# ReubenBond/DistributedRateLimiting.Redis

Measured on AMD Instinct MI355X. Metric: acquire decisions/sec (node) at 100M keys, 1/2/4/8 GPU; % HBM roofline, higher is better.
Workload: dtype f64; 1 GPU; TokenBucket uniform keys, 2^26-request batches (config B); keys_total=100000000, keys_per_gpu=100000000, batch_per_gpu=67108864, period_ticks=10000000, partitioning=one GPU owns every key

## Files before the change

__graft_entry__.py:

```python
from __future__ import annotations

import os
import sys

ROOT = os.path.dirname(os.path.abspath(__file__))
if ROOT not in sys.path:
    sys.path.insert(0, ROOT)


def build() -> None:
    import importlib.util

    spec = importlib.util.spec_from_file_location(
        "_tbe_build", os.path.join(ROOT, "distributedratelimiting.redis_amd", "build.py"))
    mod = importlib.util.module_from_spec(spec)
    spec.loader.exec_module(mod)
    mod.build_engine(verbose=True)
    mod.build_host(verbose=True)
    from oracle.build import build_oracle

    build_oracle()
    spec = importlib.util.spec_from_file_location(
        "_host_test", os.path.join(ROOT, "tests", "test_host_cpp.py"))
    tmod = importlib.util.module_from_spec(spec)
    spec.loader.exec_module(tmod)
    tmod.build_host_test()
    import distributedratelimiting.redis_amd


def smoke() -> None:
    import numpy as np
    import torch

    from distributedratelimiting.redis_amd import TokenBucketEngine
    from oracle import cref, trace

    assert torch.cuda.is_available(), "smoke() needs a GPU"
    torch.cuda.set_device(0)
    n_keys, n = 10_000, 50_000
    token_limit, tokens_per_period, period_ticks = 20, 10, 10_000_000
    eng = TokenBucketEngine(n_keys, token_limit, tokens_per_period, period_ticks, device=0)
    ref = cref.CTokenBucket(n_keys, token_limit, eng_rate(tokens_per_period, period_ticks))
    for b in range(3):
        keys, permits, ts = trace.make_batch(0x5EED0001, n_keys, b, n, 200_000, 1, 3)
        g, r = eng.acquire_batch(keys, permits, ts)
        g_ref, r_ref = ref.acquire_batch(keys, permits, ts)
        assert np.array_equal(g, g_ref), f"granted mismatch in batch {b}"
        assert np.array_equal(r, r_ref), f"remaining mismatch in batch {b}"
    v, t = eng.export_state()
    v_ref, t_ref = ref.export_state()
    touched = t_ref != np.iinfo(np.int64).min
    assert np.array_equal(t, t_ref)
    assert np.array_equal(v[touched].view(np.uint64), v_ref[touched].view(np.uint64))
    eng.close()
    print(f"smoke ok: {3 * n} decisions bit-exact vs oracle, grant rate {g.mean():.3f}")


def eng_rate(tokens_per_period: int, period_ticks: int) -> float:
    from distributedratelimiting.redis_amd import fill_rate

    return fill_rate(tokens_per_period, period_ticks)


if __name__ == "__main__":
    build()
    if len(sys.argv) > 1 and sys.argv[1] == "smoke":
        smoke()
```

distributedratelimiting.redis_amd/build.py:

```python
from __future__ import annotations

import os
import shutil
import subprocess
import sys

HERE = os.path.dirname(os.path.realpath(__file__))
ROOT = os.path.dirname(HERE)
SOURCES = [os.path.join(HERE, "csrc", n) for n in ("tbe_engine.hip", "tbe_tools.hip", "tbe_cluster.hip", "tbe_strdir.hip")]
DEPS = SOURCES + [os.path.join(HERE, "csrc", n) for n in ("tbe_device.hpp", "tbe_codec.hpp", "tbe_numfmt.hpp", "tbe_hash.hpp")] + \
    [os.path.join(ROOT, "include", n) for n in ("tbe.h", "tbe_tools.h", "tbe_cluster.h", "tbe_strdir.h")]
LIB = os.path.join(HERE, "libtbe.so")
ARCH = "gfx950"
HIPCC_FLAGS = ["-O3", "-std=c++17", "-ffp-contract=off", "-fno-fast-math", "-fPIC", "-shared",
               "-Wall", "-Wno-unused-result", f"--offload-arch={ARCH}"]


def hipcc() -> str:
    for cand in (os.environ.get("HIPCC"), shutil.which("hipcc"), "/opt/rocm/bin/hipcc"):
        if cand and os.path.exists(cand):
            return cand
    raise FileNotFoundError("hipcc not found")


def _digest(deps, flags) -> str:
    import hashlib
    h = hashlib.sha256(" ".join(flags).encode())
    for d in deps:
        with open(d, "rb") as f:
            h.update(os.path.basename(d).encode() + b"\0" + f.read())
    return h.hexdigest()


def up_to_date(target: str, deps, flags=()) -> bool:
    stamp = target + ".sha256"
    if not (os.path.exists(target) and os.path.exists(stamp)):
        return False
    with open(stamp) as f:
        return f.read().strip() == _digest(deps, flags)


def _stamp(target: str, deps, flags=()) -> None:
    with open(target + ".sha256", "w") as f:
        f.write(_digest(deps, flags) + "\n")


def build_engine(force: bool = False, verbose: bool = False, defines=(), out: str = LIB) -> str:
    flags = HIPCC_FLAGS + [f"-D{d}" for d in defines]
    if not force and up_to_date(out, DEPS, flags):
        if verbose:
            print(f"build: {os.path.basename(out)} up to date (sources sha256 {_digest(DEPS, flags)[:12]})",
                  file=sys.stderr)
        return out
    cmd = [hipcc()] + flags + ["-I", os.path.join(ROOT, "include"), "-o", out + ".tmp"] + SOURCES
    if verbose:
        print(" ".join(cmd), file=sys.stderr)
    subprocess.run(cmd, check=True)
    os.replace(out + ".tmp", out)
    _stamp(out, DEPS, flags)
    return out


HOST_SRC = os.path.join(HERE, "host", "rate_limiting.cpp")
HOST_DEPS = [HOST_SRC, os.path.join(HERE, "host", "rate_limiting.hpp"), os.path.join(ROOT, "include", "tbe.h")]
HOST_LIB = os.path.join(HERE, "libtbe_host.so")
CXX_FLAGS = ["-O2", "-std=c++17", "-Wall", "-Wextra", "-Wno-unused-parameter", "-pthread"]


def build_host(force: bool = False, verbose: bool = False) -> str:
    build_engine(verbose=verbose)
    if not force and up_to_date(HOST_LIB, HOST_DEPS + [LIB], CXX_FLAGS):
        return HOST_LIB
    cmd = ["g++"] + CXX_FLAGS + ["-fPIC", "-shared", "-I", os.path.join(ROOT, "include"),
                                 "-o", HOST_LIB + ".tmp", HOST_SRC, "-L", HERE, "-ltbe",
                                 "-Wl,-rpath,$ORIGIN"]
    if verbose:
        print(" ".join(cmd), file=sys.stderr)
    subprocess.run(cmd, check=True)
    os.replace(HOST_LIB + ".tmp", HOST_LIB)
    _stamp(HOST_LIB, HOST_DEPS + [LIB], CXX_FLAGS)
    return HOST_LIB


if __name__ == "__main__":
    print(build_engine(force="--force" in sys.argv, verbose=True))
    print(build_host(force="--force" in sys.argv, verbose=True))
```

distributedratelimiting.redis_amd/csrc/tbe_codec.hpp:

```cpp
#pragma once
#include <cstdint>

#if defined(__HIPCC__)
#define TBE_CODEC_FN __host__ __device__ __forceinline__
#else
#define TBE_CODEC_FN inline
#endif

struct PackFmt {
    uint64_t kmask;
    int32_t kb;
    int32_t pb;
    int32_t pc_max;
    int32_t wb;
    int32_t n0;
    int32_t rb;
    int32_t w0;
};
TBE_CODEC_FN uint32_t pack_rec32(uint32_t pkey, int32_t p, int64_t ts, int64_t tbase, const PackFmt &F, bool &esc) {
    const uint32_t pc = (uint32_t)(p < 0 ? 0 : (p > F.pc_max ? F.pc_max : p));
    const uint64_t d = (uint64_t)ts - (uint64_t)tbase;
    const bool fits = ts >= tbase && (d >> F.w0) == 0;
    esc = !fits;
    return (pkey & ((1u << F.rb) - 1u)) | (pc << F.rb) | ((uint32_t)!fits << (F.rb + F.pb)) |
           (fits ? (uint32_t)d << (F.rb + F.pb + 1) : 0u);
}

struct FoldFmt {
    int32_t on;
    int32_t n0;
    int32_t rb, pb, pw, tw;
    uint32_t nb;
    uint32_t region_bits;
    uint32_t n_hi;
};
TBE_CODEC_FN uint64_t fold_rec32(uint32_t r32, uint32_t pos, int64_t tbase0, int64_t tbase1, const PackFmt &F,
                           const FoldFmt &G) {
    const uint64_t row = r32 & ((1u << F.rb) - 1u);
    const uint64_t pc = (r32 >> F.rb) & ((1u << F.pb) - 1u);
    const bool esc0 = (r32 >> (F.rb + F.pb)) & 1u;
    const int64_t ts = (int64_t)((uint64_t)tbase0 + (uint64_t)(r32 >> (F.rb + F.pb + 1)));
    const uint64_t d = (uint64_t)ts - (uint64_t)tbase1;
    const bool fits = !esc0 && ts >= tbase1 && (d >> G.tw) == 0;
    return row | (pc << G.rb) | ((uint64_t)!fits << (G.rb + G.pb)) | ((uint64_t)pos << (G.rb + G.pb + 1)) |
           ((fits ? d : 0ull) << (G.rb + G.pb + 1 + G.pw));
}

struct Pass1Codec {
    uint32_t low_mask;
    uint32_t s_esc;
    uint32_t s_pos;
    uint32_t s_time;
    uint64_t dconst;
};
TBE_CODEC_FN bool pass1_codec_ok(const PackFmt &F, const FoldFmt &G) {
    return F.n0 && G.pw >= 1 && G.pw <= 32 && F.rb == G.rb && F.pb == G.pb && F.w0 == 32 - F.rb - F.pb - 1 &&
           F.w0 >= 1 && G.tw == 64 - G.rb - G.pb - 1 - G.pw && G.tw >= F.w0;
}
TBE_CODEC_FN Pass1Codec pass1_codec(const PackFmt &F, const FoldFmt &G, bool have_ts) {
    Pass1Codec C;
    C.s_esc = (uint32_t)(F.rb + F.pb);
    C.s_pos = C.s_esc + 1u;
    C.s_time = C.s_pos + (uint32_t)G.pw;
    C.low_mask = (1u << C.s_pos) - 1u;
    C.dconst = have_ts ? (1ull << (G.tw - 1)) - (1ull << (F.w0 - 1)) : 0ull;
    return C;
}
TBE_CODEC_FN uint64_t fold_rec32_codec(uint32_t r32, uint32_t pos, const Pass1Codec &C) {
    const bool esc0 = (r32 >> C.s_esc) & 1u;
    const uint64_t d = (uint64_t)(r32 >> C.s_pos) + C.dconst;
    const uint32_t plo = pos << C.s_pos, phi = pos >> (32u - C.s_pos);
    return ((uint64_t)phi << 32 | ((r32 & C.low_mask) | plo)) | ((esc0 ? 0ull : d) << C.s_time);
}
```

distributedratelimiting.redis_amd/csrc/tbe_device.hpp:

```cpp
#pragma once

#include <hip/hip_runtime.h>
#include <stdint.h>

#pragma clang fp contract(off)

namespace tbe {

constexpr int kBlock = 256;
constexpr int kWaves = kBlock / 64;
constexpr int kDigitBits = 8;
constexpr int kDigits = 1 << kDigitBits;
constexpr int64_t kAbsent = INT64_MIN;

struct __attribute__((aligned(16))) Slot {
    double v;
    int64_t t_us;
};

__device__ __forceinline__ double lua_max(double a, double b) { return (b > a) ? b : a; }
__device__ __forceinline__ double lua_min(double a, double b) { return (b < a) ? b : a; }

__device__ __forceinline__ void split_ts(int64_t ts_us, int64_t &sec, int64_t &usec) {
    int64_t s = (int64_t)((double)ts_us * 1e-6);
    int64_t r = ts_us - s * 1000000;
    if (r < 0) {
        s -= 1;
        r += 1000000;
    } else if (r >= 1000000) {
        s += 1;
        r -= 1000000;
    }
    sec = s;
    usec = r;
}

__device__ __forceinline__ double new_t_of(int64_t ts_us) {
    int64_t sec, usec;
    split_ts(ts_us, sec, usec);
    const double x = (double)usec;
    const double rcp = 1.0 / 1000000.0;
    const double q0 = x * rcp;
    const double r = __builtin_fma(-q0, 1000000.0, x);
    const double q = __builtin_fma(r, rcp, q0);
    return (double)sec + q;
}

struct TbParams {
    double cap;
    double rate;
    int64_t ttl_ms;
};

struct ReqTime {
    double new_t;
    int64_t exp_lt;
    int64_t ts;
};
__device__ __forceinline__ ReqTime req_time(int64_t ts_us, int64_t ttl_ms) {
    ReqTime r;
    r.new_t = new_t_of(ts_us);
    r.exp_lt = (ts_us / 1000 - ttl_ms) * 1000;
    r.ts = ts_us;
    return r;
}

struct TimeBase {
    int64_t tbase;
    int64_t e0;
    uint32_t sec0;
    uint32_t usec0;
    uint32_t r0;
    uint32_t ok;
};
constexpr uint64_t kRelMax = 0xFFFFFFFFull - 1000000ull;
__host__ __device__ inline TimeBase time_base(int64_t tbase, int64_t ttl_ms) {
    TimeBase b{tbase, 0, 0, 0, 0, 0};
    if (tbase < 0) return b;
    const int64_t sec0 = tbase / 1000000;
    if (sec0 > (int64_t)0xFFFFFFFFll - 10000) return b;
    b.sec0 = (uint32_t)sec0;
    b.usec0 = (uint32_t)(tbase - sec0 * 1000000);
    b.r0 = (uint32_t)(tbase % 1000);
    b.e0 = (tbase / 1000 - ttl_ms) * 1000;
    b.ok = 1;
    return b;
}
__device__ __forceinline__ ReqTime req_time_rel(int64_t ts_us, const TimeBase &B, int64_t ttl_ms) {
    const uint64_t d = (uint64_t)ts_us - (uint64_t)B.tbase;
    if (!B.ok || ts_us < B.tbase || d > kRelMax) return req_time(ts_us, ttl_ms);
    const uint32_t u = B.usec0 + (uint32_t)d;
    const uint32_t s1 = u / 1000000u;
    const uint32_t usec = u - s1 * 1000000u;
    const uint32_t sec = B.sec0 + s1;
    const double x = (double)usec;
    const double rcp = 1.0 / 1000000.0;
    const double q0 = x * rcp;
    const double r = __builtin_fma(-q0, 1000000.0, x);
    const double q = __builtin_fma(r, rcp, q0);
    ReqTime rt;
    rt.new_t = (double)sec + q;
    rt.exp_lt = B.e0 + (int64_t)((B.r0 + (uint32_t)d) / 1000u) * 1000;
    rt.ts = ts_us;
    return rt;
}
#ifndef TBE_ABSENT_BASE
#define TBE_ABSENT_BASE 1
#endif
__device__ __forceinline__ int64_t absent_t(const TimeBase &B) { return TBE_ABSENT_BASE ? B.tbase : 0; }

__device__ __forceinline__ uint32_t tb_step_ft(Slot &row, double ft, int32_t permits,
                                               const ReqTime &rq, const TbParams &P, bool &modified) {
    const bool had = row.t_us != kAbsent;
    const bool expired = had && row.t_us < rq.exp_lt;
    const bool present = had && !expired;
    const double pv = present ? row.v : P.cap;
    const double pt = present ? ft : rq.new_t;
    const double delta_t = lua_max(0.0, rq.new_t - pt);
    const double fill = delta_t * P.rate;
    double x = lua_max(0.0, lua_min(P.cap, pv + fill));
    const double p = (double)permits;
    const bool granted = x >= p;
    if (granted) {
        x = x - p;
        row.v = x;
        row.t_us = rq.ts;
    } else if (expired) {
        row.v = P.cap;
        row.t_us = kAbsent;
    }
    modified = granted || expired;
    return (granted ? 0x80000000u : 0u) | (uint32_t)(int32_t)x;
}

__device__ __forceinline__ uint32_t tb_step(Slot &row, int32_t permits, const ReqTime &rq,
                                            const TbParams &P, bool &modified) {
    const double ft = new_t_of(row.t_us == kAbsent ? 0 : row.t_us);
    return tb_step_ft(row, ft, permits, rq, P, modified);
}

__device__ __forceinline__ uint32_t tb_acquire(Slot &s, int32_t permits, int64_t ts_us,
                                               const TbParams &P, bool &modified) {
    return tb_step(s, permits, req_time(ts_us, P.ttl_ms), P, modified);
}

template <typename T>
__device__ __forceinline__ T ld_nt(const T *p) { return __builtin_nontemporal_load(p); }
template <typename T>
__device__ __forceinline__ void st_nt(T *p, T v) { __builtin_nontemporal_store(v, p); }

__device__ __forceinline__ uint32_t xcd_swizzle(uint32_t b, uint32_t nblk) {
    const uint32_t xcd = b & 7u, q = nblk >> 3, r = nblk & 7u;
    return (xcd < r ? xcd * (q + 1) : r * (q + 1) + (xcd - r) * q) + (b >> 3);
}

__device__ __forceinline__ uint64_t lanemask_lt() {
    const int lane = threadIdx.x & 63;
    return (lane == 0) ? 0ull : ((~0ull) >> (64 - lane));
}

template <int BLOCK>
__device__ __forceinline__ uint32_t block_excl_scan(uint32_t x, uint32_t *wsum, uint32_t *total) {
    constexpr int W = BLOCK / 64;
    const int lane = threadIdx.x & 63, w = threadIdx.x >> 6;
    uint32_t v = x;
#pragma unroll
    for (int o = 1; o < 64; o <<= 1) {
        const uint32_t y = __shfl_up(v, o, 64);
        if (lane >= o) v += y;
    }
    if (lane == 63) wsum[w] = v;
    __syncthreads();
    uint32_t pre = 0, tot = 0;
#pragma unroll
    for (int j = 0; j < W; ++j) {
        const uint32_t s = wsum[j];
        pre += (j < w) ? s : 0u;
        tot += s;
    }
    *total = tot;
    __syncthreads();
    return pre + v - x;
}

#ifndef TBE_WAVE_MATCH
#define TBE_WAVE_MATCH 1
#endif
__device__ __forceinline__ uint64_t digit_peers(uint32_t key, int shift, uint64_t vmask) {
#if TBE_WAVE_MATCH
    const uint32_t dg = (key >> shift) & (kDigits - 1);
    uint32_t dlo = 0, dhi = 0;
#pragma unroll
    for (int b = 0; b < kDigitBits; ++b) {
        const uint32_t sb = (uint32_t)__builtin_amdgcn_sbfe((int)dg, (uint32_t)b, 1u);
        const uint64_t m = __builtin_amdgcn_uicmp(sb, 0u, 33);
        dlo |= (uint32_t)m ^ sb;
        dhi |= (uint32_t)(m >> 32) ^ sb;
    }
    return vmask & ~(((uint64_t)dhi << 32) | dlo);
#else
    const uint32_t dg = (key >> shift) & (kDigits - 1);
    uint64_t peers = vmask;
#pragma unroll
    for (int b = 0; b < kDigitBits; ++b) {
        const bool bit = (dg >> b) & 1u;
        const uint64_t m = __ballot(bit);
        peers &= bit ? m : ~m;
    }
    return peers;
#endif
}

template <int BLOCK>
struct RankLds {
    static constexpr int W = BLOCK / 64;
    static constexpr int PARTS = BLOCK / kDigits;
    uint32_t lstart[kDigits];
    uint32_t part[PARTS][kDigits];
    uint32_t wsum[W];
};

template <int BLOCK, int ITEMS>
__device__ __forceinline__ void rank_tile(const uint32_t (&key)[ITEMS], int shift, int nvalid,
                                          RankLds<BLOCK> &L, uint16_t *cnt,
                                          uint32_t (&lpos)[ITEMS]) {
#define TBE_DIG(it) ((key[it] >> shift) & (kDigits - 1))
    constexpr int W = BLOCK / 64;
    constexpr int COL = ITEMS * W;
    static_assert(BLOCK % kDigits == 0, "whole digit columns per thread group");
    const int tid = threadIdx.x, w = tid >> 6;
    {
        uint4 *z = reinterpret_cast<uint4 *>(cnt);
        const uint4 zero = {0u, 0u, 0u, 0u};
        for (int i = tid; i < COL * kDigits * 2 / 16; i += BLOCK) z[i] = zero;
    }
    __syncthreads();
    const uint64_t lt = lanemask_lt();
#pragma unroll
    for (int it = 0; it < ITEMS; ++it) {
        const int e = it * BLOCK + tid;
        const bool valid = e < nvalid;
        const uint32_t dg = TBE_DIG(it);
        const uint64_t peers = digit_peers(key[it], shift, __ballot(valid));
        lpos[it] = (uint32_t)__popcll(peers & lt);
        if (valid && lpos[it] == 0) cnt[(it * W + w) * kDigits + dg] = (uint16_t)__popcll(peers);
    }
    __syncthreads();
    constexpr int PARTS = BLOCK / kDigits;
    static_assert(COL % PARTS == 0, "column splits evenly");
    constexpr int SEG = COL / PARTS;
    const int d = tid & (kDigits - 1);
    const int part = tid / kDigits;
    uint32_t s = 0;
#pragma unroll 8
    for (int j = part * SEG; j < (part + 1) * SEG; ++j) {
        const uint32_t c = cnt[j * kDigits + d];
        cnt[j * kDigits + d] = (uint16_t)s;
        s += c;
    }
    L.part[part][d] = s;
    __syncthreads();
    uint32_t off = 0, total = 0;
#pragma unroll
    for (int q = 0; q < PARTS; ++q) {
        const uint32_t v = L.part[q][d];
        off += (q < part) ? v : 0u;
        total += v;
    }
    if (part > 0) {
#pragma unroll 8
        for (int j = part * SEG; j < (part + 1) * SEG; ++j)
            cnt[j * kDigits + d] = (uint16_t)(cnt[j * kDigits + d] + off);
    }
    {
        uint32_t all;
        const uint32_t ex = block_excl_scan<BLOCK>(part == 0 ? total : 0u, L.wsum, &all);
        if (part == 0) L.lstart[d] = ex;
    }
    __syncthreads();
#pragma unroll
    for (int it = 0; it < ITEMS; ++it)
        lpos[it] += L.lstart[TBE_DIG(it)] + cnt[(it * W + w) * kDigits + TBE_DIG(it)];
#undef TBE_DIG
}

template <int BLOCK, int ITEMS>
__device__ __forceinline__ int wb_elem(int it) {
    return (int)((threadIdx.x >> 6) * (64 * ITEMS) + it * 64 + (threadIdx.x & 63));
}

template <int BLOCK, int ITEMS, bool FULL = false>
__device__ __forceinline__ void rank_tile_wb(const uint32_t (&key)[ITEMS], int shift, int nvalid,
                                             RankLds<BLOCK> &L, uint32_t *wcnt, uint32_t (&lpos)[ITEMS]) {
    constexpr int W = BLOCK / 64;
    const int tid = threadIdx.x, w = tid >> 6, lane = tid & 63;
    uint32_t *mine = wcnt + w * kDigits;
#pragma unroll
    for (int i = lane; i < kDigits; i += 64) mine[i] = 0;
    __builtin_amdgcn_fence(__ATOMIC_RELEASE, "wavefront");
    const uint64_t lt = lanemask_lt();
#pragma unroll
    for (int it = 0; it < ITEMS; ++it) {
        const int e = wb_elem<BLOCK, ITEMS>(it);
        const bool valid = FULL || e < nvalid;
        const uint32_t dg = (key[it] >> shift) & (kDigits - 1);
        const uint64_t peers = digit_peers(key[it], shift, FULL ? ~0ull : __ballot(valid));
        const int leader = (FULL || peers) ? __ffsll((long long)peers) - 1 : lane;
        uint32_t old = 0;
        if (valid && leader == lane) old = atomicAdd(&mine[dg], (uint32_t)__popcll(peers));
        old = __shfl(old, leader, 64);
        lpos[it] = old + (uint32_t)__popcll(peers & lt);
    }
    __syncthreads();
    uint32_t tot = 0;
    if (tid < kDigits) {
#pragma unroll
        for (int v = 0; v < W; ++v) {
            const uint32_t c = wcnt[v * kDigits + tid];
            wcnt[v * kDigits + tid] = tot;
            tot += c;
        }
    }
    {
        uint32_t all;
        const uint32_t ex = block_excl_scan<BLOCK>(tid < kDigits ? tot : 0u, L.wsum, &all);
        if (tid < kDigits) L.lstart[tid] = ex;
    }
    __syncthreads();
#pragma unroll
    for (int it = 0; it < ITEMS; ++it) {
        const uint32_t dg = (key[it] >> shift) & (kDigits - 1);
        lpos[it] += L.lstart[dg] + mine[dg];
    }
}

}
```

distributedratelimiting.redis_amd/csrc/tbe_engine.hip:

```cpp
#include <hip/hip_runtime.h>

#include <algorithm>
#include <cmath>
#include <cstdarg>
#include <cstdio>
#include <cstdlib>
#include <cstring>
#include <new>
#include <string>
#include <thread>
#include <tuple>
#include <type_traits>
#include <vector>

#include "../../include/tbe.h"
#include "tbe_device.hpp"
#include "tbe_codec.hpp"
#include "tbe_numfmt.hpp"

#pragma clang fp contract(off)

using namespace tbe;

namespace {

#ifndef TBE_NO_NT
#define LD_P(p) ld_nt(p)
#define ST_PERM(p, v) st_nt((p), (v))
#define LD_U(p) ld_nt(p)
#define ST_U(p, v) st_nt((p), (v))
#define ST_S(p, v) slot_store_nt((p), (v))
#else
#define LD_P(p) (*(p))
#define ST_PERM(p, v) (*(p) = (v))
#define LD_U(p) (*(p))
#define ST_U(p, v) (*(p) = (v))
#define ST_S(p, v) (*(p) = (v))
#endif
#define LD_F(p) (*(p))
#define ST_F(p, v) (*(p) = (v))

#ifndef TBE_PART_BLOCK
#define TBE_PART_BLOCK 512
#endif
#ifndef TBE_PART_ITEMS
#define TBE_PART_ITEMS 8
#endif
constexpr int kPartBlock = TBE_PART_BLOCK;
constexpr int kPartItems = TBE_PART_ITEMS;
constexpr int kTile = kPartBlock * kPartItems;
#ifndef TBE_UN_BLOCK
#define TBE_UN_BLOCK 1024
#endif
#ifndef TBE_UN_ITEMS
#define TBE_UN_ITEMS 8
#endif
constexpr int kUnBlock = TBE_UN_BLOCK;
constexpr int kUnItems = TBE_UN_ITEMS;
constexpr int kUnTile = kUnBlock * kUnItems;
#ifndef TBE_FULL_TILE
#define TBE_FULL_TILE 1
#endif
#ifndef TBE_HIST_BLOCKS
#define TBE_HIST_BLOCKS 1024
#endif
constexpr int kMaxHistBlocks = TBE_HIST_BLOCKS;
static_assert(kMaxHistBlocks % 256 == 0, "k_colscan reads kMaxHistBlocks / 256 blocks per thread");
constexpr int kMaxRBits = 11;

constexpr uint32_t kHotKeysMax = 1024;
#ifndef TBE_HOT_SLOT_BITS
#define TBE_HOT_SLOT_BITS 12
#endif
constexpr uint32_t kHotSlots = 1u << TBE_HOT_SLOT_BITS;
static_assert(kHotSlots >= 2 * kHotKeysMax, "hot table load factor <= 1/2");
constexpr uint32_t kHotEmpty = 0xFFFFFFFFu;
constexpr uint32_t kHotMin = 2048;
constexpr uint32_t kHotCandMax = 4096;

struct HotSet {
    uint32_t count;
    uint32_t n_cand;
    uint32_t key[kHotKeysMax];
    uint64_t cand[kHotCandMax];
    uint64_t slot[kHotSlots];
};

__device__ __forceinline__ uint32_t hot_hash(uint32_t key) { return (key * 0x9E3779B1u) >> (32 - TBE_HOT_SLOT_BITS); }
constexpr uint64_t kHotSlotEmpty = 0xFFFFFFFFFFFFFFFFull;
constexpr uint32_t kHotHalf = kHotSlots / 2;
__device__ __forceinline__ uint32_t hot_h1(uint32_t key) { return (key * 0x9E3779B1u) >> (33 - TBE_HOT_SLOT_BITS); }
__device__ __forceinline__ uint32_t hot_h2(uint32_t key) {
    uint32_t x = (key ^ (key >> 16)) * 0x85EBCA6Bu;
    x ^= x >> 13;
    return kHotHalf + ((x * 0xC2B2AE35u) >> (33 - TBE_HOT_SLOT_BITS));
}

constexpr uint32_t kHotLds = kHotSlots;
template <int BLOCK>
__device__ __forceinline__ bool hot_load(const HotSet *__restrict__ hot, uint64_t *slots) {
    const bool any = hot != nullptr && hot->count != 0;
    if (any)
        for (int j = threadIdx.x; j < (int)kHotSlots; j += BLOCK) slots[j] = hot->slot[j];
    __syncthreads();
    return any;
}
__device__ __forceinline__ const uint64_t *hot_table(const HotSet *__restrict__, const uint64_t *lds) {
    return lds;
}

__device__ __forceinline__ uint32_t hot_sortkey(uint32_t key, const uint64_t *slots, uint32_t nb,
                                                int r_bits) {
    const uint64_t v1 = slots[hot_h1(key)], v2 = slots[hot_h2(key)];
    if ((uint32_t)v1 == key) return (nb + (uint32_t)(v1 >> 32)) << r_bits;
    if ((uint32_t)v2 == key) return (nb + (uint32_t)(v2 >> 32)) << r_bits;
    return key;
    uint32_t h = hot_hash(key);
    for (;;) {
        const uint64_t v = slots[h];
        const uint32_t k = (uint32_t)v;
        if (k == key) return (nb + (uint32_t)(v >> 32)) << r_bits;
        if (k == kHotEmpty) return key;
        h = (h + 1) & (kHotSlots - 1);
    }
}

template <int N, typename KeyT>
__device__ __forceinline__ void hot_sortkeys(const KeyT (&kv)[N], const uint64_t *slots, uint32_t nb,
                                             int r_bits, uint32_t (&sk)[N]) {
    constexpr int G = N < 4 ? N : 4;
    static_assert(N % G == 0, "groups of G requests");
#pragma unroll
    for (int g = 0; g < N; g += G) {
        uint64_t v1[G], v2[G];
#pragma unroll
        for (int u = 0; u < G; ++u) {
            v1[u] = slots[hot_h1((uint32_t)kv[g + u])];
            v2[u] = slots[hot_h2((uint32_t)kv[g + u])];
        }
#pragma unroll
        for (int u = 0; u < G; ++u) {
            const uint32_t key = (uint32_t)kv[g + u];
            const bool in1 = (uint32_t)v1[u] == key;
            const uint64_t v = in1 ? v1[u] : v2[u];
            sk[g + u] = (in1 || (uint32_t)v2[u] == key) ? (nb + (uint32_t)(v >> 32)) << r_bits : key;
        }
    }
    return;
    uint64_t v[N];
#pragma unroll
    for (int it = 0; it < N; ++it) v[it] = slots[hot_hash((uint32_t)kv[it])];
#pragma unroll
    for (int it = 0; it < N; ++it) {
        const uint32_t key = (uint32_t)kv[it];
        const uint32_t k = (uint32_t)v[it];
        if (k == key) sk[it] = (nb + (uint32_t)(v[it] >> 32)) << r_bits;
        else if (k == kHotEmpty) sk[it] = key;
        else sk[it] = hot_sortkey(key, slots, nb, r_bits);
    }
}

constexpr int kHBlock = 512;
constexpr int kHItems = kTile / kHBlock;
#ifndef TBE_HIST_AHEAD
#define TBE_HIST_AHEAD 1
#endif
#ifndef TBE_HIST_WAVES
#define TBE_HIST_WAVES 8
#endif
#ifndef TBE_HIST_HOT_WAVES
#define TBE_HIST_HOT_WAVES 6
#endif
template <typename KeyT, bool HOT = false>
__global__ __launch_bounds__(kHBlock, HOT ? TBE_HIST_HOT_WAVES : TBE_HIST_WAVES) void k_hist(const KeyT *__restrict__ keys, uint64_t n,
                                                  int shift, uint32_t tiles_per_blk,
                                                  uint32_t ntiles, uint32_t *__restrict__ tileprefix,
                                                  uint32_t *__restrict__ blocksum, uint64_t n_keys,
                                                  uint32_t *__restrict__ err, int validate,
                                                  uint64_t kmask, const HotSet *__restrict__ hot = nullptr,
                                                  uint32_t nb = 0, int r_bits = 0,
                                                  uint32_t *__restrict__ bcount = nullptr,
                                                  int lowbits = 0, uint32_t nbt = 0,
                                                  uint8_t *__restrict__ dig_out = nullptr) {
    __shared__ uint32_t h8[kDigits * 8];
    __shared__ uint32_t tile_lo[2];
    static_assert(kHBlock == 2 * kDigits && kDigits * 8 == 4 * kHBlock, "two threads per digit; 4 counters each");
    __shared__ uint64_t hs[HOT ? kHotLds : 1];
    const int tid = threadIdx.x;
    const bool dig = tid < kDigits;
    const bool any_hot = HOT && hot_load<kHBlock>(hot, hs);
    const uint32_t t0 = blockIdx.x * tiles_per_blk;
    const uint32_t t1 = min(t0 + tiles_per_blk, ntiles);
    uint32_t run = 0;
    uint32_t acc = 0, acc_lo = 0;
    bool bad = false;
    KeyT kn[kHItems];
#if TBE_HIST_AHEAD >= 2
    KeyT kn2[kHItems];
#endif
    auto load_into = [&](KeyT (&dst)[kHItems], uint32_t t) {
#pragma unroll
        for (int it = 0; it < kHItems; ++it) {
            const uint64_t i = (uint64_t)t * kTile + it * kHBlock + tid;
            dst[it] = (t < t1 && i < n) ? LD_P(keys + i) : (KeyT)0;
        }
    };
    load_into(kn, t0);
#if TBE_HIST_AHEAD >= 2
    load_into(kn2, t0 + 1);
#endif
    for (uint32_t t = t0; t < t1; ++t) {
        KeyT kv[kHItems];
#pragma unroll
        for (int it = 0; it < kHItems; ++it) kv[it] = kn[it];
#if TBE_HIST_AHEAD >= 2
#pragma unroll
        for (int it = 0; it < kHItems; ++it) kn[it] = kn2[it];
        load_into(kn2, t + 2);
#else
        load_into(kn, t + 1);
#endif
#pragma unroll
        for (int u = 0; u < 4; ++u) h8[u * kHBlock + tid] = 0;
        __syncthreads();
        const uint64_t base = (uint64_t)t * kTile;
        const uint64_t last = min<uint64_t>(base + kTile, n) - 1;
        uint32_t skv[kHItems];
        if (HOT && any_hot) {
            hot_sortkeys<kHItems>(kv, hot_table(hot, hs), nb, r_bits, skv);
        } else {
#pragma unroll
            for (int it = 0; it < kHItems; ++it) skv[it] = (uint32_t)((uint64_t)kv[it] & kmask);
        }
#pragma unroll
        for (int it = 0; it < kHItems; ++it) {
            const uint64_t i = base + it * kHBlock + tid;
            const bool valid = i < n;
            const uint32_t sk = skv[it];
            const uint32_t d = (sk >> shift) & (kDigits - 1);
            const uint64_t vmask = __ballot(valid);
            const uint32_t d0 = __shfl(d, vmask ? __ffsll((long long)vmask) - 1 : 0, 64);
            if (__all(!valid || d == d0)) {
                if (vmask && (vmask & lanemask_lt()) == 0 && valid) atomicAdd(&h8[d0 * 8], (uint32_t)__popcll(vmask));
            } else {
                if (valid) atomicAdd(&h8[d * 8 + (tid & 7)], 1u);
            }
            if (dig_out && valid) dig_out[i] = (uint8_t)d;
            if (valid) {
                bad |= validate && ((uint64_t)kv[it] >= n_keys);
                if (bcount && (i == base || i == last)) {
                    tile_lo[i == last] = lowbits ? (sk >> r_bits) & ((1u << lowbits) - 1u) : 0u;
                    if (i == base && i == last) tile_lo[0] = tile_lo[1];
                }
            }
        }
        __syncthreads();
        uint32_t c = 0;
        if (dig) {
#pragma unroll
            for (int u = 0; u < 8; ++u) c += h8[tid * 8 + ((u + tid) & 7)];
            tileprefix[(uint64_t)t * kDigits + tid] = run;
            run += c;
        }
        if (bcount) {
            const uint32_t lo0 = tile_lo[0], lo1 = tile_lo[1];
            if (lo0 == lo1) {
                if (dig) {
                    if (lo0 != acc_lo) {
                        const uint32_t bk = ((uint32_t)tid << lowbits) | acc_lo;
                        if (acc && bk < nbt) atomicAdd(&bcount[bk], acc);
                        acc = 0;
                        acc_lo = lo0;
                    }
                    acc += c;
                }
            } else if (lo1 - lo0 < 8) {
                __syncthreads();
#pragma unroll
                for (int u = 0; u < 4; ++u) h8[u * kHBlock + tid] = 0;
                __syncthreads();
#pragma unroll
                for (int it = 0; it < kHItems; ++it) {
                    const uint64_t i = base + it * kHBlock + tid;
                    const uint32_t bk = skv[it] >> r_bits;
                    if (i < n) atomicAdd(&h8[((bk & ((1u << lowbits) - 1u)) - lo0) * kDigits + ((bk >> lowbits) & (kDigits - 1))], 1u);
                }
                __syncthreads();
                if (dig) {
                    for (uint32_t u = 0; u <= lo1 - lo0; ++u) {
                        const uint32_t cnt = h8[u * kDigits + tid];
                        const uint32_t bk = ((uint32_t)tid << lowbits) | (lo0 + u);
                        if (cnt && bk < nbt) atomicAdd(&bcount[bk], cnt);
                    }
                }
            } else {
#pragma unroll
                for (int it = 0; it < kHItems; ++it) {
                    const uint64_t i = base + it * kHBlock + tid;
                    const uint32_t bk = skv[it] >> r_bits;
                    if (i < n && bk < nbt) atomicAdd(&bcount[bk], 1u);
                }
            }
        }
        __syncthreads();
    }
    if (bcount && dig) {
        const uint32_t bk = ((uint32_t)tid << lowbits) | acc_lo;
        if (acc && bk < nbt) atomicAdd(&bcount[bk], acc);
    }
    if (dig) blocksum[(uint64_t)blockIdx.x * kDigits + tid] = run;
    if (__any(bad) && (tid & 63) == 0) atomicOr(err, 1u);
}

__global__ __launch_bounds__(kHBlock, TBE_HIST_WAVES) void k_hist_dig(
    const uint8_t *__restrict__ dig, uint64_t n, uint32_t tiles_per_blk, uint32_t ntiles,
    uint32_t *__restrict__ tileprefix, uint32_t *__restrict__ blocksum,
    const uint32_t *__restrict__ dtot0, uint32_t *__restrict__ bcount, uint32_t nbt) {
    __shared__ uint32_t h8[kDigits * 8];
    __shared__ uint32_t dstart[kDigits + 1];
    __shared__ uint32_t wsum[kHBlock / 64];
    __shared__ uint32_t tlo[kHBlock];
    static_assert(kHBlock == 2 * kDigits && kDigits * 8 == 4 * kHBlock, "two threads per digit; 4 counters each");
    static_assert(kHItems % 8 == 0, "8-byte loads");
    constexpr int kW = kHItems / 8;
    const int tid = threadIdx.x;
    const bool own = tid < kDigits;
    {
        uint32_t all;
        const uint32_t pre = block_excl_scan<kHBlock>(own ? dtot0[tid] : 0u, wsum, &all);
        if (own) dstart[tid] = pre;
        if (tid == 0) dstart[kDigits] = 0xFFFFFFFFu;
    }
    auto d0_of = [&](uint32_t i) {
        uint32_t lo = 0, hi = kDigits;
        while (hi - lo > 1) {
            const uint32_t mid = (lo + hi) >> 1;
            if (dstart[mid] <= i) lo = mid;
            else hi = mid;
        }
        return lo;
    };
    const uint32_t t0 = blockIdx.x * tiles_per_blk;
    const uint32_t t1 = min(t0 + tiles_per_blk, ntiles);
    uint32_t run = 0, acc = 0, acc_lo = 0;
    auto load = [&](uint32_t t, uint64_t (&dst)[kW]) {
#pragma unroll
        for (int q = 0; q < kW; ++q) {
            const uint64_t i = (uint64_t)t * kTile + (uint64_t)tid * kHItems + 8 * q;
            uint64_t v = 0;
            if (t < t1 && i + 8 <= n) {
                v = LD_P(reinterpret_cast<const uint64_t *>(dig + i));
            } else if (t < t1) {
                for (int u = 0; i + u < n; ++u) v |= (uint64_t)dig[i + u] << (8 * u);
            }
            dst[q] = v;
        }
    };
    uint64_t vn[kW];
    load(t0, vn);
    __syncthreads();
    for (uint32_t t = t0; t < t1; ++t) {
        uint64_t vw[kW];
#pragma unroll
        for (int q = 0; q < kW; ++q) vw[q] = vn[q];
        load(t + 1, vn);
#pragma unroll
        for (int u = 0; u < 4; ++u) h8[u * kHBlock + tid] = 0;
        const uint64_t base = (uint64_t)t * kTile;
        const uint32_t tk = (t - t0) % (kHBlock / 2);
        if (tk == 0) {
            const uint32_t tt = t + (uint32_t)(tid >> 1);
            if (tt < t1) {
                const uint64_t b = (uint64_t)tt * kTile;
                tlo[tid] = d0_of((uint32_t)((tid & 1) ? min<uint64_t>(b + kTile, n) - 1 : b));
            }
        }
        __syncthreads();
        if (TBE_FULL_TILE && base + kTile <= n) {
#pragma unroll
            for (int u = 0; u < kHItems; ++u) {
                const uint32_t d = (uint32_t)(vw[u >> 3] >> (8 * (u & 7))) & (kDigits - 1);
                const uint32_t dw = (uint32_t)__builtin_amdgcn_readfirstlane((int)d);
                if (__all(d == dw)) {
                    if ((tid & 63) == 0) atomicAdd(&h8[dw * 8], 64u);
                } else {
                    atomicAdd(&h8[d * 8 + (tid & 7)], 1u);
                }
            }
        } else {
            const uint32_t nv = (uint32_t)(n - base);
#pragma unroll
            for (int u = 0; u < kHItems; ++u) {
                const bool valid = (uint32_t)(tid * kHItems + u) < nv;
                const uint32_t d = (uint32_t)(vw[u >> 3] >> (8 * (u & 7))) & (kDigits - 1);
                const uint64_t vmask = __ballot(valid);
                const uint32_t dw = __shfl(d, vmask ? __ffsll((long long)vmask) - 1 : 0, 64);
                if (__all(!valid || d == dw)) {
                    if (vmask && (vmask & lanemask_lt()) == 0 && valid) atomicAdd(&h8[dw * 8], (uint32_t)__popcll(vmask));
                } else if (valid) {
                    atomicAdd(&h8[d * 8 + (tid & 7)], 1u);
                }
            }
        }
        __syncthreads();
        uint32_t c = 0;
        if (own) {
#pragma unroll
            for (int u = 0; u < 8; ++u) c += h8[tid * 8 + ((u + tid) & 7)];
            tileprefix[(uint64_t)t * kDigits + tid] = run;
            run += c;
        }
        const uint32_t lo0 = tlo[2 * tk], lo1 = tlo[2 * tk + 1];
        if (lo0 == lo1) {
            if (own) {
                if (lo0 != acc_lo) {
                    const uint32_t bk = ((uint32_t)tid << kDigitBits) | acc_lo;
                    if (acc && bk < nbt) atomicAdd(&bcount[bk], acc);
                    acc = 0;
                    acc_lo = lo0;
                }
                acc += c;
            }
        } else if (lo1 - lo0 < 8) {
            __syncthreads();
#pragma unroll
            for (int u = 0; u < 4; ++u) h8[u * kHBlock + tid] = 0;
            __syncthreads();
#pragma unroll
            for (int u = 0; u < kHItems; ++u) {
                const uint64_t i = base + (uint64_t)tid * kHItems + u;
                if (i >= n) continue;
                uint32_t lo = 0;
                for (uint32_t x = 1; x <= lo1 - lo0; ++x) lo += dstart[lo0 + x] <= (uint32_t)i;
                const uint32_t d = (uint32_t)(vw[u >> 3] >> (8 * (u & 7))) & (kDigits - 1);
                atomicAdd(&h8[lo * kDigits + d], 1u);
            }
            __syncthreads();
            if (own) {
                for (uint32_t u = 0; u <= lo1 - lo0; ++u) {
                    const uint32_t cnt = h8[u * kDigits + tid];
                    const uint32_t bk = ((uint32_t)tid << kDigitBits) | (lo0 + u);
                    if (cnt && bk < nbt) atomicAdd(&bcount[bk], cnt);
                }
            }
        } else {
#pragma unroll
            for (int u = 0; u < kHItems; ++u) {
                const uint64_t i = base + (uint64_t)tid * kHItems + u;
                if (i >= n) continue;
                const uint32_t bk = (((uint32_t)(vw[u >> 3] >> (8 * (u & 7))) & (kDigits - 1)) << kDigitBits) | d0_of((uint32_t)i);
                if (bk < nbt) atomicAdd(&bcount[bk], 1u);
            }
        }
        __syncthreads();
    }
    if (own) {
        const uint32_t bk = ((uint32_t)tid << kDigitBits) | acc_lo;
        if (acc && bk < nbt) atomicAdd(&bcount[bk], acc);
        blocksum[(uint64_t)blockIdx.x * kDigits + tid] = run;
    }
}

__global__ __launch_bounds__(kBlock) void k_colscan(const uint32_t *__restrict__ blocksum,
                                                    uint32_t nblk,
                                                    uint32_t *__restrict__ blockprefix,
                                                    uint32_t *__restrict__ digit_total) {
    __shared__ uint32_t wsum[kWaves];
    const int d = blockIdx.x, tid = threadIdx.x;
    constexpr int PER = kMaxHistBlocks / kBlock;
    uint32_t c[PER], s = 0;
#pragma unroll
    for (int u = 0; u < PER; ++u) {
        const uint32_t j = tid * PER + u;
        c[u] = (j < nblk) ? blocksum[(uint64_t)j * kDigits + d] : 0u;
        s += c[u];
    }
    uint32_t total;
    uint32_t pre = block_excl_scan<kBlock>(s, wsum, &total);
#pragma unroll
    for (int u = 0; u < PER; ++u) {
        const uint32_t j = tid * PER + u;
        if (j < nblk) blockprefix[(uint64_t)j * kDigits + d] = pre;
        pre += c[u];
    }
    if (tid == 0) digit_total[d] = total;
}

template <int BLOCK>
__device__ __forceinline__ void tile_offsets(uint32_t tile, uint32_t tiles_per_blk,
                                             const uint32_t *__restrict__ tileprefix,
                                             const uint32_t *__restrict__ blockprefix,
                                             const uint32_t *__restrict__ digit_total,
                                             uint32_t *goff, uint32_t *wsum) {
    const int tid = threadIdx.x;
    uint32_t tot = (tid < kDigits) ? digit_total[tid] : 0u;
    uint32_t all;
    const uint32_t base = block_excl_scan<BLOCK>(tot, wsum, &all);
    if (tid < kDigits)
        goff[tid] = base + blockprefix[(uint64_t)(tile / tiles_per_blk) * kDigits + tid] +
                    tileprefix[(uint64_t)tile * kDigits + tid];
}

template <typename KeyIn, bool IDX, bool TS = true>
__global__ __launch_bounds__(kPartBlock) void k_scatter(
    const KeyIn *__restrict__ kin, const int32_t *__restrict__ pin, const int64_t *__restrict__ tin,
    const uint32_t *__restrict__ iin, uint64_t n, int shift, const uint32_t *__restrict__ tileprefix,
    const uint32_t *__restrict__ blockprefix, const uint32_t *__restrict__ digit_total,
    uint32_t tiles_per_blk, uint32_t *__restrict__ kout, int32_t *__restrict__ pout,
    int64_t *__restrict__ tout, uint32_t *__restrict__ iout, uint32_t *__restrict__ perm,
    uint32_t *__restrict__ err, int validate) {
    __shared__ RankLds<kPartBlock> L;
    __shared__ uint32_t goff[kDigits];
    __shared__ uint64_t stage[kTile];
    static_assert(kPartItems * (kPartBlock / 64) * kDigits * 2 <= kTile * 8, "cnt fits in stage");

    const int tid = threadIdx.x;
    const uint32_t tile = xcd_swizzle(blockIdx.x, gridDim.x);
    const uint64_t base = (uint64_t)tile * kTile;
    const int nvalid = (int)min<uint64_t>(kTile, n - base);

    uint32_t key[kPartItems], lpos[kPartItems];
    int32_t pm[kPartItems];
    int64_t tv[kPartItems];
#pragma unroll
    for (int it = 0; it < kPartItems; ++it) {
        const int e = it * kPartBlock + tid;
        const bool v = e < nvalid;
        key[it] = v ? (uint32_t)kin[base + e] : 0u;
        pm[it] = v ? pin[base + e] : 0;
        tv[it] = (v && TS) ? tin[base + e] : 0;
    }
    tile_offsets<kPartBlock>(tile, tiles_per_blk, tileprefix, blockprefix, digit_total, goff, L.wsum);
    rank_tile<kPartBlock, kPartItems>(key, shift, nvalid, L, reinterpret_cast<uint16_t *>(stage), lpos);
    __syncthreads();

    bool bad = false;
#pragma unroll
    for (int it = 0; it < kPartItems; ++it) {
        const int e = it * kPartBlock + tid;
        if (e < nvalid) {
            const uint32_t d = (key[it] >> shift) & (kDigits - 1);
            bad |= validate && (pm[it] < 0 || tv[it] < 0);
            stage[lpos[it]] = ((uint64_t)key[it] << 32) | (uint32_t)pm[it];
            perm[base + e] = goff[d] + lpos[it] - L.lstart[d];
        }
    }
    __syncthreads();
    uint32_t gpos[kPartItems];
#pragma unroll
    for (int it = 0; it < kPartItems; ++it) {
        const int j = it * kPartBlock + tid;
        if (j < nvalid) {
            const uint64_t s = stage[j];
            const uint32_t k = (uint32_t)(s >> 32);
            const uint32_t d = (k >> shift) & (kDigits - 1);
            gpos[it] = goff[d] + (uint32_t)j - L.lstart[d];
            kout[gpos[it]] = k;
            pout[gpos[it]] = (int32_t)(uint32_t)s;
        }
    }
    if (TS) {
        __syncthreads();
#pragma unroll
        for (int it = 0; it < kPartItems; ++it) {
            const int e = it * kPartBlock + tid;
            if (e < nvalid) stage[lpos[it]] = (uint64_t)tv[it];
        }
        __syncthreads();
#pragma unroll
        for (int it = 0; it < kPartItems; ++it) {
            const int j = it * kPartBlock + tid;
            if (j < nvalid) tout[gpos[it]] = (int64_t)stage[j];
        }
    }
    if (IDX) {
        uint32_t *stage32 = reinterpret_cast<uint32_t *>(stage);
        uint32_t iv[kPartItems];
#pragma unroll
        for (int it = 0; it < kPartItems; ++it) {
            const int e = it * kPartBlock + tid;
            iv[it] = (e < nvalid) ? (iin ? iin[base + e] : (uint32_t)(base + e)) : 0u;
        }
        __syncthreads();
#pragma unroll
        for (int it = 0; it < kPartItems; ++it) {
            const int e = it * kPartBlock + tid;
            if (e < nvalid) stage32[lpos[it]] = iv[it];
        }
        __syncthreads();
#pragma unroll
        for (int it = 0; it < kPartItems; ++it) {
            const int j = it * kPartBlock + tid;
            if (j < nvalid) iout[gpos[it]] = stage32[j];
        }
    }
    if (validate && __any(bad) && (tid & 63) == 0) atomicOr(err, 1u);
}

constexpr int kScanPer = 16;
__global__ __launch_bounds__(1024) void k_bscan(const uint32_t *__restrict__ bcount, uint32_t nbt,
                                                uint32_t *__restrict__ bstart, uint32_t nb = 0,
                                                uint32_t wide_min = 0, uint32_t *__restrict__ dlist = nullptr) {
    __shared__ uint32_t tile[1024 * (kScanPer + 1)];
    auto pad = [](uint32_t j) { return (j / kScanPer) * (kScanPer + 1) + (j % kScanPer); };
    __shared__ uint32_t wsum[16];
    __shared__ uint32_t n_dense;
    if (threadIdx.x == 0) n_dense = 0;
    const uint32_t t = threadIdx.x;
    constexpr uint32_t kRow = 1024 * kScanPer;
    constexpr int kGroup = 4;
    uint32_t carry = 0;
    for (uint32_t g0 = 0; g0 < nbt; g0 += kGroup * kRow) {
        uint32_t ld[kGroup][kScanPer];
#pragma unroll
        for (int r = 0; r < kGroup; ++r)
#pragma unroll
            for (int k = 0; k < kScanPer; ++k) {
                const uint32_t j = g0 + r * kRow + k * 1024 + t;
                ld[r][k] = j < nbt ? bcount[j] : 0u;
            }
#pragma unroll
        for (int r = 0; r < kGroup; ++r) {
            const uint32_t r0 = g0 + r * kRow;
            if (r0 >= nbt) break;
#pragma unroll
            for (int k = 0; k < kScanPer; ++k) tile[pad(k * 1024 + t)] = ld[r][k];
            __syncthreads();
            uint32_t v[kScanPer], sum = 0;
#pragma unroll
            for (int k = 0; k < kScanPer; ++k) {
                v[k] = tile[t * (kScanPer + 1) + k];
                sum += v[k];
            }
            if (dlist) {
#pragma unroll
                for (int k = 0; k < kScanPer; ++k) {
                    const uint32_t bk = r0 + t * kScanPer + k;
                    if (bk < nb && v[k] >= wide_min) dlist[1 + atomicAdd(&n_dense, 1u)] = bk;
                }
            }
            uint32_t total;
            uint32_t pre = carry + block_excl_scan<1024>(sum, wsum, &total);
#pragma unroll
            for (int k = 0; k < kScanPer; ++k) {
                tile[t * (kScanPer + 1) + k] = pre;
                pre += v[k];
            }
            __syncthreads();
#pragma unroll
            for (int k = 0; k < kScanPer; ++k) {
                const uint32_t j = r0 + k * 1024 + t;
                if (j < nbt) bstart[j] = tile[pad(k * 1024 + t)];
            }
            carry += total;
            __syncthreads();
        }
    }
    if (t == 0) bstart[nbt] = carry;
    if (dlist) {
        __syncthreads();
        if (t == 0) dlist[0] = n_dense;
    }
}

constexpr int kBsPer = 4;
constexpr uint32_t kBsTile = 1024u * kBsPer;
constexpr uint32_t kBsMaxBlocks = 64;
__global__ __launch_bounds__(1024) void k_bscan_lb(const uint32_t *__restrict__ bcount, uint32_t nbt,
                                                   uint32_t *__restrict__ bstart,
                                                   unsigned long long *__restrict__ flags, uint32_t tag,
                                                   uint32_t nb = 0, uint32_t wide_min = 0,
                                                   uint32_t *__restrict__ dlist = nullptr) {
    __shared__ uint32_t wsum[16];
    __shared__ uint32_t excl;
    const uint32_t t = threadIdx.x, blk = blockIdx.x;
    const uint32_t b0 = blk * kBsTile + t * kBsPer;
    uint32_t v[kBsPer];
#pragma unroll
    for (int k = 0; k < kBsPer; ++k) v[k] = (b0 + k < nbt) ? bcount[b0 + k] : 0u;
    if (dlist) {
#pragma unroll
        for (int k = 0; k < kBsPer; ++k)
            if (b0 + k < nb && v[k] >= wide_min) dlist[1 + atomicAdd(dlist, 1u)] = b0 + k;
    }
    uint32_t sum = 0;
#pragma unroll
    for (int k = 0; k < kBsPer; ++k) sum += v[k];
    uint32_t total;
    const uint32_t pre = block_excl_scan<1024>(sum, wsum, &total);
    if (t == 0)
        __hip_atomic_store(&flags[blk], ((unsigned long long)tag << 32) | total, __ATOMIC_RELEASE,
                           __HIP_MEMORY_SCOPE_AGENT);
    if (t < 64) {
        uint32_t acc = 0;
        for (uint32_t j0 = 0; j0 < blk; j0 += 64) {
            const uint32_t j = j0 + t;
            uint32_t val = 0;
            if (j < blk) {
                unsigned long long f;
                do {
                    f = __hip_atomic_load(&flags[j], __ATOMIC_ACQUIRE, __HIP_MEMORY_SCOPE_AGENT);
                } while ((uint32_t)(f >> 32) != tag);
                val = (uint32_t)f;
            }
#pragma unroll
            for (int o = 32; o > 0; o >>= 1) val += __shfl_xor(val, o, 64);
            acc += val;
        }
        if (t == 0) excl = acc;
    }
    __syncthreads();
    uint32_t run = excl + pre;
#pragma unroll
    for (int k = 0; k < kBsPer; ++k) {
        if (b0 + k < nbt) bstart[b0 + k] = run;
        run += v[k];
    }
    if (blk == gridDim.x - 1 && t == 0) bstart[nbt] = excl + total;
}

__device__ __forceinline__ int64_t pack_base32(const int64_t *__restrict__ ts, const PackFmt &F) {
    return ts[0] - ((int64_t)1 << (F.w0 - 1));
}
__device__ __forceinline__ int64_t pack_base(const int64_t *__restrict__ ts, const PackFmt &F) {
    return ts[0] - ((int64_t)1 << (F.wb - 1));
}
#ifndef TBE_REL_BASE
#define TBE_REL_BASE 1
#endif
__device__ __forceinline__ int64_t rel_base(const int64_t *__restrict__ ts, const PackFmt &F) {
#if TBE_REL_BASE
    (void)F;
    const int64_t b = ts[0] - ((int64_t)1 << 31);
    return b > 0 ? b : 0;
#else
    return pack_base(ts, F);
#endif
}
__device__ __forceinline__ uint64_t pack_rec(uint64_t key, int32_t p, int64_t ts, uint64_t idx,
                                             int64_t tbase, const PackFmt &F) {
    const uint64_t pc = (uint64_t)(p < 0 ? 0 : (p > F.pc_max ? F.pc_max : p));
    const uint64_t d = (uint64_t)ts - (uint64_t)tbase;
    const bool fits = ts >= tbase && (d >> F.wb) == 0;
    const uint64_t pay = fits ? d : idx;
    return (key & F.kmask) | (pc << F.kb) | ((uint64_t)!fits << (F.kb + F.pb)) |
           (pay << (F.kb + F.pb + 1));
}
__device__ __forceinline__ void unpack_rec(uint64_t rec, const int64_t *__restrict__ ts_orig,
                                           int64_t tbase, const PackFmt &F, uint32_t &key,
                                           int32_t &p, int64_t &ts) {
    key = (uint32_t)(rec & F.kmask);
    p = (int32_t)((rec >> F.kb) & ((1ull << F.pb) - 1));
    const uint64_t pay = rec >> (F.kb + F.pb + 1);
    ts = ((rec >> (F.kb + F.pb)) & 1) ? ts_orig[pay] : (int64_t)((uint64_t)tbase + pay);
}

__device__ __forceinline__ int64_t fold_base(const int64_t *__restrict__ ts, const FoldFmt &G) {
    return ts[0] - ((int64_t)1 << (G.tw - 1));
}
__device__ __forceinline__ uint64_t fold_rec(uint64_t rec0, uint32_t pos, int64_t tbase0, int64_t tbase1,
                                             const PackFmt &F, const FoldFmt &G) {
    const uint64_t row = rec0 & ((1ull << G.rb) - 1);
    const uint64_t pc = (rec0 >> F.kb) & ((1ull << F.pb) - 1);
    const bool esc0 = (rec0 >> (F.kb + F.pb)) & 1;
    const int64_t ts = (int64_t)((uint64_t)tbase0 + (rec0 >> (F.kb + F.pb + 1)));
    const uint64_t d = (uint64_t)ts - (uint64_t)tbase1;
    const bool fits = !esc0 && ts >= tbase1 && (d >> G.tw) == 0;
    return row | (pc << G.rb) | ((uint64_t)!fits << (G.rb + G.pb)) | ((uint64_t)pos << (G.rb + G.pb + 1)) |
           ((fits ? d : 0ull) << (G.rb + G.pb + 1 + G.pw));
}
__device__ __forceinline__ void unfold_rec(uint64_t rec, const FoldFmt &G, int64_t tbase1,
                                           const uint64_t *__restrict__ rec0, const int64_t *__restrict__ ts_orig,
                                           int64_t tbase0, const PackFmt &F, uint32_t &row, int32_t &p,
                                           int64_t &ts, uint32_t &pos) {
    row = (uint32_t)(rec & ((1ull << G.rb) - 1));
    p = (int32_t)((rec >> G.rb) & ((1ull << G.pb) - 1));
    pos = (uint32_t)((rec >> (G.rb + G.pb + 1)) & ((1ull << G.pw) - 1));
    if ((rec >> (G.rb + G.pb)) & 1) {
        if (G.n0) {
            ts = (int64_t)rec0[pos];
        } else {
            uint32_t k;
            int32_t p0;
            unpack_rec(rec0[pos], ts_orig, tbase0, F, k, p0, ts);
        }
    } else {
        ts = (int64_t)((uint64_t)tbase1 + (rec >> (G.rb + G.pb + 1 + G.pw)));
    }
}
__device__ __forceinline__ uint32_t fold_bucket_at(const FoldFmt &G, uint32_t blk) {
    if (!G.on) return blk;
    const uint32_t x = blk & 7u, s = blk >> 3;
    const uint32_t j = s / G.n_hi, hi = s - j * G.n_hi;
    return (hi << G.region_bits) | (x + 8u * j);
}
__device__ __forceinline__ uint32_t fold_bucket(const FoldFmt &G) { return fold_bucket_at(G, blockIdx.x); }
__device__ __forceinline__ void fold_input(uint64_t rec, uint32_t q, const FoldFmt &G, int64_t tbase1,
                                           const uint64_t *__restrict__ rec0, const int64_t *__restrict__ ts_orig,
                                           int64_t tbase0, const PackFmt &F, uint32_t rmask, uint32_t &row,
                                           int32_t &p, int64_t &ts, uint32_t &pos) {
    if (G.on) {
        unfold_rec(rec, G, tbase1, rec0, ts_orig, tbase0, F, row, p, ts, pos);
    } else {
        uint32_t k;
        unpack_rec(rec, ts_orig, tbase0, F, k, p, ts);
        row = k & rmask;
        pos = q;
    }
}

#ifndef TBE_FOLD_FAM
#define TBE_FOLD_FAM 1
#endif
template <int FAM>
__device__ __forceinline__ void fold_input_fam(uint64_t rec, uint32_t q, const FoldFmt &G, int64_t tbase1,
                                               const uint64_t *__restrict__ rec0,
                                               const int64_t *__restrict__ ts_orig, int64_t tbase0,
                                               const PackFmt &F, uint32_t rmask, uint32_t &row, int32_t &p,
                                               int64_t &ts, uint32_t &pos) {
    if (FAM < 0) {
        fold_input(rec, q, G, tbase1, rec0, ts_orig, tbase0, F, rmask, row, p, ts, pos);
    } else if (FAM == 0) {
        uint32_t k;
        unpack_rec(rec, ts_orig, tbase0, F, k, p, ts);
        row = k & rmask;
        pos = q;
    } else {
        row = (uint32_t)(rec & ((1ull << G.rb) - 1));
        p = (int32_t)((rec >> G.rb) & ((1ull << G.pb) - 1));
        pos = (uint32_t)((rec >> (G.rb + G.pb + 1)) & ((1ull << G.pw) - 1));
        if ((rec >> (G.rb + G.pb)) & 1) {
            if (FAM == 1) {
                ts = (int64_t)rec0[pos];
            } else {
                uint32_t k;
                int32_t p0;
                unpack_rec(rec0[pos], ts_orig, tbase0, F, k, p0, ts);
            }
        } else {
            ts = (int64_t)((uint64_t)tbase1 + (rec >> (G.rb + G.pb + 1 + G.pw)));
        }
    }
}

#ifndef TBE_BSCAN_LB
#define TBE_BSCAN_LB 1
#endif
#ifndef TBE_NARROW0
#define TBE_NARROW0 1
#endif
#ifndef TBE_SCATTER0_WAVES
#define TBE_SCATTER0_WAVES 1
#endif
#ifndef TBE_PASS1_CODEC
#define TBE_PASS1_CODEC 1
#endif
constexpr int kLastWaves = 3 * (kPartBlock / 64) / 4;
template <bool FIRST, bool HOT = false, bool IDX = false, bool NOTS = false, bool LAST = false, int FAM = -1>
__global__ __launch_bounds__(kPartBlock, FIRST ? TBE_SCATTER0_WAVES : (FAM >= 0 ? kLastWaves : 1)) void k_scatter_rec(
    const uint64_t *__restrict__ kin, const int32_t *__restrict__ pin, const int64_t *__restrict__ tin,
    const uint64_t *__restrict__ rin, uint64_t n, int shift, PackFmt F,
    const uint32_t *__restrict__ tileprefix, const uint32_t *__restrict__ blockprefix,
    const uint32_t *__restrict__ digit_total, uint32_t tiles_per_blk, uint64_t *__restrict__ rout,
    uint32_t *__restrict__ perm, uint32_t *__restrict__ err, const HotSet *__restrict__ hot = nullptr,
    uint32_t nb = 0, int r_bits = 0, const uint32_t *__restrict__ iin = nullptr,
    uint32_t *__restrict__ iout = nullptr, FoldFmt G = FoldFmt{}, uint8_t *__restrict__ dig_next = nullptr,
    const uint8_t *__restrict__ din = nullptr, int64_t *__restrict__ ts0 = nullptr, Pass1Codec C = Pass1Codec{}) {
    static_assert(!(FIRST && LAST), "fold records come from a pass after the first");
    static_assert(FAM < 0 || LAST, "the record family is fixed only for the last pass");
    const bool n0 = FAM < 0 ? F.n0 != 0 : FAM == 1;
    __shared__ RankLds<kPartBlock> L;
    __shared__ uint32_t goff[kDigits];
    __shared__ uint64_t stage[kTile];
    __shared__ uint16_t stage_e[LAST ? kTile : 1];
    __shared__ uint64_t hs[HOT ? kHotLds : 1];
    static_assert(kPartItems * (kPartBlock / 64) * kDigits * 2 <= kTile * 8, "cnt fits in stage");

    const int tid = threadIdx.x;
    const uint32_t tile = xcd_swizzle(blockIdx.x, gridDim.x);
    const uint64_t base = (uint64_t)tile * kTile;
    const int nv = (int)min((uint32_t)kTile, (uint32_t)(n - base));

    auto body = [&](auto full) {
        constexpr bool FULL = decltype(full)::value;
        const int nvalid = nv;
        uint64_t rec[kPartItems];
        uint32_t key[kPartItems], lpos[kPartItems];
        bool bad = false;
        bool any_hot = false;
        int64_t tv_keep[FIRST ? kPartItems : 1];
        if (FIRST) {
            uint64_t kv[kPartItems];
            int32_t pv[kPartItems];
            int64_t tv[kPartItems];
#pragma unroll
            for (int it = 0; it < kPartItems; ++it) {
                const int e = wb_elem<kPartBlock, kPartItems>(it);
                const bool v = (FULL || e < nvalid);
                kv[it] = v ? LD_P(kin + base + e) : 0ull;
                pv[it] = v ? LD_P(pin + base + e) : 0;
                tv[it] = NOTS ? -1 : (v ? LD_P(tin + base + e) : 0);
            }
            any_hot = HOT && hot_load<kPartBlock>(hot, hs);
            const int64_t tbase = NOTS ? 0 : (n0 ? pack_base32(tin, F) : pack_base(tin, F));
            uint32_t skv[kPartItems];
            if (HOT && any_hot) {
                hot_sortkeys<kPartItems>(kv, hot_table(hot, hs), nb, r_bits, skv);
            } else {
#pragma unroll
                for (int it = 0; it < kPartItems; ++it) skv[it] = (uint32_t)(kv[it] & F.kmask);
            }
#pragma unroll
            for (int it = 0; it < kPartItems; ++it) {
                const int e = wb_elem<kPartBlock, kPartItems>(it);
                bad |= (FULL || e < nvalid) && (pv[it] < 0 || (!NOTS && tv[it] < 0));
                if (n0) {
                    bool esc = false;
                    const uint32_t r32 =
                        NOTS ? (skv[it] & ((1u << F.rb) - 1u)) |
                                   ((uint32_t)(pv[it] < 0 ? 0 : (pv[it] > F.pc_max ? F.pc_max : pv[it])) << F.rb)
                             : pack_rec32(skv[it], pv[it], tv[it], tbase, F, esc);
                    rec[it] = (uint64_t)r32 | ((uint64_t)((skv[it] >> shift) & (kDigits - 1)) << 32) |
                              ((uint64_t)((skv[it] >> (shift + kDigitBits)) & (kDigits - 1)) << 40) |
                              ((uint64_t)esc << 48);
                } else {
                    rec[it] = pack_rec(skv[it], pv[it], tv[it], base + e, tbase, F);
                }
                key[it] = skv[it];
                tv_keep[FIRST ? it : 0] = tv[it];
            }
        } else {
            if (n0) {
                const uint32_t *rin32 = reinterpret_cast<const uint32_t *>(rin);
                uint8_t dv[kPartItems];
#pragma unroll
                for (int it = 0; it < kPartItems; ++it) {
                    const int e = wb_elem<kPartBlock, kPartItems>(it);
                    rec[it] = (FULL || e < nvalid) ? (uint64_t)LD_P(rin32 + base + e) : 0ull;
                    dv[it] = (FULL || e < nvalid) ? din[base + e] : (uint8_t)0;
                }
#pragma unroll
                for (int it = 0; it < kPartItems; ++it) {
                    key[it] = (uint32_t)dv[it] << shift;
                    rec[it] |= (uint64_t)dv[it] << 32;
                }
            } else {
#pragma unroll
                for (int it = 0; it < kPartItems; ++it) {
                    const int e = wb_elem<kPartBlock, kPartItems>(it);
                    rec[it] = (FULL || e < nvalid) ? LD_P(rin + base + e) : 0ull;
                    key[it] = (uint32_t)(rec[it] & F.kmask);
                }
            }
        }
        tile_offsets<kPartBlock>(tile, tiles_per_blk, tileprefix, blockprefix, digit_total, goff, L.wsum);
        rank_tile_wb<kPartBlock, kPartItems, FULL>(key, shift, nvalid, L, reinterpret_cast<uint32_t *>(stage), lpos);
        int64_t tbase0 = 0, tbase1 = 0;
        if (LAST && FAM != 1 && tin) {
            tbase0 = n0 ? pack_base32(tin, F) : pack_base(tin, F);
            tbase1 = fold_base(tin, G);
        }
        __syncthreads();
#pragma unroll
        for (int it = 0; it < kPartItems; ++it) {
            const int e = wb_elem<kPartBlock, kPartItems>(it);
            if (FULL || e < nvalid) {
                const uint32_t d = (key[it] >> shift) & (kDigits - 1);
                stage[lpos[it]] = n0 ? (rec[it] & 0x0000FFFFFFFFFFFFull) : rec[it];
                if (LAST)
                    stage_e[lpos[it]] = (uint16_t)e;
                else if (perm)
                    ST_PERM(perm + base + e, goff[d] + lpos[it] - L.lstart[d]);
                if (FIRST && n0 && ((rec[it] >> 48) & 1u))
                    ts0[goff[d] + lpos[it] - L.lstart[d]] = tv_keep[FIRST ? it : 0];
            }
        }
        __syncthreads();
        uint32_t gpos[kPartItems];
#pragma unroll
        for (int it = 0; it < kPartItems; ++it) {
            const int j = it * kPartBlock + tid;
            if (FULL || j < nvalid) {
                const uint64_t s = stage[j];
                const uint32_t d = n0 ? (uint32_t)(s >> 32) & (kDigits - 1)
                                      : ((uint32_t)(s & F.kmask) >> shift) & (kDigits - 1);
                gpos[it] = goff[d] + (uint32_t)j - L.lstart[d];
                if (n0 && !LAST)
                    reinterpret_cast<uint32_t *>(rout)[gpos[it]] = (uint32_t)s;
                else if (n0)
                    rout[gpos[it]] = FAM == 1 ? fold_rec32_codec((uint32_t)s, (uint32_t)(base + stage_e[j]), C)
                                              : fold_rec32((uint32_t)s, (uint32_t)(base + stage_e[j]), tbase0, tbase1, F, G);
                else
                    rout[gpos[it]] = LAST ? fold_rec(s, (uint32_t)(base + stage_e[j]), tbase0, tbase1, F, G) : s;
                if (!LAST && dig_next)
                    dig_next[gpos[it]] = n0 ? (uint8_t)(s >> 40)
                                            : (uint8_t)(((uint32_t)(s & F.kmask) >> (shift + kDigitBits)) & (kDigits - 1));
            }
        }
        if (IDX) {
            uint32_t *stage32 = reinterpret_cast<uint32_t *>(stage);
            uint32_t iv[kPartItems];
#pragma unroll
            for (int it = 0; it < kPartItems; ++it) {
                const int e = wb_elem<kPartBlock, kPartItems>(it);
                iv[it] = (FULL || e < nvalid) ? (FIRST ? (uint32_t)(base + e) : iin[base + e]) : 0u;
            }
            __syncthreads();
#pragma unroll
            for (int it = 0; it < kPartItems; ++it) {
                const int e = wb_elem<kPartBlock, kPartItems>(it);
                if (FULL || e < nvalid) stage32[lpos[it]] = iv[it];
            }
            __syncthreads();
#pragma unroll
            for (int it = 0; it < kPartItems; ++it) {
                const int j = it * kPartBlock + tid;
                if (FULL || j < nvalid) iout[gpos[it]] = stage32[j];
            }
        }
        if (FIRST && __any(bad) && (tid & 63) == 0) atomicOr(err, 1u);
    };
    if (TBE_FULL_TILE && nv == kTile)
        body(std::true_type{});
    else
        body(std::false_type{});
}

constexpr int kFoldBlock = 512;
constexpr int kFoldPer = 4;
constexpr int kFoldChunk = kFoldBlock * kFoldPer;
constexpr int kMaxRows = 1 << kMaxRBits;

typedef uint32_t u32x4 __attribute__((ext_vector_type(4)));
__device__ __forceinline__ void slot_store_nt(Slot *p, const Slot &s) {
    u32x4 v;
    __builtin_memcpy(&v, &s, sizeof v);
    __builtin_nontemporal_store(v, reinterpret_cast<u32x4 *>(p));
}
__device__ __forceinline__ Slot slot_load_nt(const Slot *p) {
    const u32x4 v = ld_nt(reinterpret_cast<const u32x4 *>(p));
    Slot s;
    __builtin_memcpy(&s, &v, sizeof s);
    return s;
}

typedef __attribute__((address_space(1))) const void gvoid_t;
typedef __attribute__((address_space(3))) void lvoid_t;
__device__ __forceinline__ void lds_dma16(const void *src, void *lds_wave) {
    __builtin_amdgcn_global_load_lds((gvoid_t *)src, (lvoid_t *)lds_wave, 16, 0, 2);
}
__device__ __forceinline__ void lds_dma_wait() {
    asm volatile("s_waitcnt vmcnt(0)" ::: "memory");
}

__device__ __forceinline__ void put_reply(uint32_t *res, uint32_t q, uint32_t rep, uint32_t narrow) {
    if (narrow)
        reinterpret_cast<uint8_t *>(res)[q] = (uint8_t)(((rep >> 24) & 0x80u) | (rep & 0x7Fu));
    else
        res[q] = rep;
}

__device__ __forceinline__ bool row_line_dirty(const uint32_t *dirty, uint32_t j) {
    return ((dirty[j >> 5] >> (j & 24u)) & 0xFFu) != 0;
}
__device__ __forceinline__ bool row_dirty(const uint32_t *dirty, uint32_t j) {
    return (dirty[j >> 5] >> (j & 31u)) & 1u;
}

#ifndef TBE_WIDE_BLOCK
#define TBE_WIDE_BLOCK 512
#endif
#ifndef TBE_WIDE_PER
#define TBE_WIDE_PER 3
#endif
#ifndef TBE_WIDE_WAVES
#define TBE_WIDE_WAVES 6
#endif
#ifndef TBE_WIDE_TAIL
#define TBE_WIDE_TAIL 512
#endif
constexpr int kWideBlock = TBE_WIDE_BLOCK;
constexpr int kWidePer = TBE_WIDE_PER;
constexpr int kWideChunk = kWideBlock * kWidePer;
constexpr int kWideTail = TBE_WIDE_TAIL;
#ifndef TBE_WIDE_SOLO
#define TBE_WIDE_SOLO 1
#endif
constexpr uint32_t kWideSolo = TBE_WIDE_SOLO ? 64u : 0u;
#ifndef TBE_FOLD_PREFETCH
#define TBE_FOLD_PREFETCH 384
#endif
#ifndef TBE_QFOLD_PREFETCH
#define TBE_QFOLD_PREFETCH 0
#endif
#ifndef TBE_AFOLD_PREFETCH
#define TBE_AFOLD_PREFETCH 0
#endif
#ifndef TBE_FOLD_PREFETCH_MIN
#define TBE_FOLD_PREFETCH_MIN 1024
#endif
#ifndef TBE_WIDE_MIN_SHIFT
#define TBE_WIDE_MIN_SHIFT 11
#endif
constexpr int kWideMinShift = TBE_WIDE_MIN_SHIFT;
static_assert(kWideChunk <= 4096 && kWideTail <= kWideBlock, "election tags and tail list");
#define WIDE_FT_GET(j, srow) req_time_rel((srow).t_us == kAbsent ? absent_t(TB) : (srow).t_us, TB, 0).new_t
#define WIDE_FT_SET(j, v) ((void)0)

template <bool PACKED, int FAM = -1>
__global__ __launch_bounds__(kWideBlock, TBE_WIDE_WAVES) void k_fold_wide(
    const uint32_t *__restrict__ skeys, const int32_t *__restrict__ sperm,
    const int64_t *__restrict__ sts, const uint64_t *__restrict__ srec,
    const int64_t *__restrict__ ts_orig, PackFmt F, const uint32_t *__restrict__ bstart,
    int r_bits, uint64_t n_keys, Slot *__restrict__ table, TbParams P,
    uint32_t *__restrict__ res, const uint32_t *__restrict__ err, HotSet *__restrict__ hot_next,
    uint32_t narrow, uint32_t wide_min, FoldFmt G, const uint64_t *__restrict__ rec0,
    const uint32_t *__restrict__ dlist = nullptr) {
    __shared__ Slot row[kMaxRows];
    __shared__ uint64_t aux[kWideTail * 2 + kWideTail / 2];
    __shared__ uint32_t wsum[kWideBlock / 64];
    uint32_t *hcnt = reinterpret_cast<uint32_t *>(aux);
    uint32_t *t_kl_lid = reinterpret_cast<uint32_t *>(aux);
    int32_t *t_pm = reinterpret_cast<int32_t *>(aux) + kWideTail;
    int64_t *t_ts = reinterpret_cast<int64_t *>(aux) + kWideTail;
    uint32_t *t_pos = reinterpret_cast<uint32_t *>(aux + kWideTail * 2);
    static_assert(kWideTail * 2 * 8 >= kMaxRows * 4, "hcnt fits in aux");
    __shared__ uint32_t own[kMaxRows];
    __shared__ uint32_t dirty[kMaxRows / 32];

    const int tid = threadIdx.x;
    if (dlist && blockIdx.x >= dlist[0]) return;
    const uint32_t b = dlist ? dlist[1 + blockIdx.x] : fold_bucket(G);
    if (G.on && b >= G.nb) return;
    const uint32_t R = 1u << r_bits;
    const uint32_t rmask = R - 1;
    const uint64_t row0 = (uint64_t)b << r_bits;
    const uint32_t nrows = (uint32_t)min<uint64_t>(R, n_keys - row0);
    Slot *__restrict__ rows = table + row0;
    constexpr int kRowsPerThread = (kMaxRows + kWideBlock - 1) / kWideBlock;
    auto slice_dma = [&]() {
#pragma unroll
        for (int u = 0; u < kRowsPerThread; ++u) {
#if defined(TBE_FOLD_COPY_ONLY) && defined(TBE_COPY_ROWS)
            if (u * kWideBlock >= (TBE_COPY_ROWS)) break;
#endif
            const uint32_t j = tid + u * kWideBlock;
            lds_dma16(rows + (j < nrows ? j : nrows - 1), &row[u * kWideBlock + (tid & ~63)]);
        }
    };
    if (*err) return;
    const uint32_t s = bstart[b], e = bstart[b + 1];
    if (s == e) return;
    if (e - s < wide_min) return;
    const bool dense = true;
    const int64_t tbase = (PACKED && FAM != 1) ? pack_base(ts_orig, F) : 0;
    const int64_t tbase1 = (FAM < 0 ? G.on != 0 : FAM >= 1) ? fold_base(ts_orig, G) : 0;
    const TimeBase TB = time_base(PACKED ? rel_base(ts_orig, F) : 0, P.ttl_ms);
    const bool count_hot = hot_next != nullptr && (e - s) >= kHotMin;

    uint32_t kl[kWidePer];
    int32_t pm[kWidePer];
    int64_t tsv[kWidePer];
    uint32_t pos[kWidePer];
    uint32_t pend = 0;
    auto load_chunk = [&](uint32_t c) {
        pend = 0;
#pragma unroll
        for (int r = 0; r < kWidePer; ++r) {
            const uint32_t q = c + r * kWideBlock + tid;
            kl[r] = 0;
            pm[r] = 0;
            tsv[r] = 0;
            pos[r] = q;
            if (q < e) {
                if (PACKED) {
                    fold_input_fam<FAM>(LD_F(srec + q), q, G, tbase1, rec0, ts_orig, tbase, F, rmask, kl[r], pm[r],
                                        tsv[r], pos[r]);
                } else {
                    kl[r] = skeys[q] & rmask;
                    pm[r] = sperm[q];
                    tsv[r] = sts[q];
                }
                pend |= 1u << r;
            }
        }
    };

#if TBE_FOLD_PREFETCH
    uint32_t pf_sink = 0;
#endif
    load_chunk(s);
    if (dense) slice_dma();
    for (uint32_t j = tid; j < (R + 31) / 32; j += kWideBlock) dirty[j] = 0;
#ifdef TBE_FOLD_COPY_ONLY
    __syncthreads();
    for (uint32_t c = s; c < e; c += kWideChunk) {
        if (c != s) load_chunk(c);
#pragma unroll
        for (int r = 0; r < kWidePer; ++r)
            if (pend & (1u << r)) put_reply(res, pos[r], kl[r] ^ (uint32_t)pm[r] ^ (uint32_t)tsv[r], narrow);
    }
#ifndef TBE_COPY_ROWS
#define TBE_COPY_ROWS kMaxRows
#endif
    for (uint32_t j = tid; j < nrows && j < (uint32_t)(TBE_COPY_ROWS); j += kWideBlock) ST_S(rows + j, row[j]);
    return;
#endif

    for (uint32_t c = s; c < e; c += kWideChunk) {
        if (c != s) load_chunk(c);
        for (uint32_t j = tid; j < R; j += kWideBlock) own[j] = 0;
        if (count_hot && c == s)
            for (uint32_t j = tid; j < R; j += kWideBlock) hcnt[j] = 0;
        lds_dma_wait();
        __syncthreads();
#if TBE_FOLD_PREFETCH
        if (c == s && e - s >= TBE_FOLD_PREFETCH_MIN) {
            const uint32_t fblk = blockIdx.x + TBE_FOLD_PREFETCH;
            const uint32_t fb = fold_bucket_at(G, fblk);
            if (fblk < gridDim.x && (!G.on || fb < G.nb)) {
                const uint32_t fs = bstart[fb], fe = bstart[fb + 1];
                if (fe - fs >= wide_min && fe > fs) {
                    if (tid < (int)(kMaxRows / 8)) {
                        const uint64_t fr = ((uint64_t)fb << r_bits) + (uint64_t)tid * 8u;
                        if (fr < n_keys) pf_sink = reinterpret_cast<const uint32_t *>(table + fr)[0];
                    } else if (PACKED) {
                        const uint32_t q = fs + (uint32_t)(tid - kMaxRows / 8) * 16u;
                        if (q < fe) pf_sink = (uint32_t)srec[q];
                    }
                }
            }
        }
#endif
        if (count_hot) {
#pragma unroll
            for (int r = 0; r < kWidePer; ++r)
                if (pend & (1u << r)) atomicAdd(&hcnt[kl[r]], 1u);
        }
        uint32_t rep[kWidePer];
#pragma unroll
        for (int r = 0; r < kWidePer; ++r) rep[r] = 0;
        auto eval_slots = [&](uint32_t round, Slot (&nrow)[kWidePer]) {
#pragma unroll
            for (int r = 0; r < kWidePer; ++r) {
                nrow[r] = Slot{0.0, 0};
                if (pend & (1u << r)) {
                    nrow[r] = row[kl[r]];
                    bool m;
                    const ReqTime rqr = PACKED ? req_time_rel(tsv[r], TB, P.ttl_ms) : req_time(tsv[r], P.ttl_ms);
                    rep[r] = tb_step_ft(nrow[r], WIDE_FT_GET(kl[r], nrow[r]), pm[r], rqr, P, m);
                    if (m) atomicMax(&own[kl[r]], (round << 12) | (4095u - (uint32_t)(r * kWideBlock + tid)));
                }
            }
        };
        auto resolve_slots = [&](uint32_t round, const Slot (&nrow)[kWidePer]) {
#pragma unroll
            for (int r = 0; r < kWidePer; ++r) {
                if (!(pend & (1u << r))) continue;
                const uint32_t tag = (round << 12) | (4095u - (uint32_t)(r * kWideBlock + tid));
                const uint32_t o = own[kl[r]];
                if ((o >> 12) != round || o < tag) {
                    pend &= ~(1u << r);
                } else if (o == tag) {
                    row[kl[r]] = nrow[r];
                    WIDE_FT_SET(kl[r], rq[r].new_t);
                    atomicOr(&dirty[kl[r] >> 5], 1u << (kl[r] & 31));
                    pend &= ~(1u << r);
                }
            }
        };
        {
            Slot nrow[kWidePer];
            eval_slots(1u, nrow);
            __syncthreads();
            resolve_slots(1u, nrow);
        }
#ifdef TBE_FOLD_R1_ONLY
        pend = 0;
#endif
        uint32_t n_tail;
        const uint32_t tail_at = block_excl_scan<kWideBlock>(__popc(pend), wsum, &n_tail);
        uint32_t keep = ~0u;
        if (n_tail != 0 && n_tail <= kWideTail && !count_hot) {
            uint32_t at = tail_at;
#pragma unroll
            for (int r = 0; r < kWidePer; ++r) {
                if (pend & (1u << r)) {
                    t_kl_lid[at] = kl[r] | ((uint32_t)(r * kWideBlock + tid) << 16);
                    t_pm[at] = pm[r];
                    t_ts[at] = tsv[r];
                    t_pos[at] = pos[r];
                    ++at;
                }
            }
            keep = ~pend;
            pend = 0;
            __syncthreads();
            bool tp = (uint32_t)tid < n_tail;
            uint32_t tkl = 0, tlid = 0, trep = 0, tpos = 0;
            int32_t tpm = 0;
            int64_t tts = 0;
            ReqTime trq{0.0, 0, 0};
            auto take = [&](uint32_t at) {
                tkl = t_kl_lid[at] & 0xFFFFu;
                tlid = t_kl_lid[at] >> 16;
                tpm = t_pm[at];
                tts = t_ts[at];
                tpos = t_pos[at];
                trq = PACKED ? req_time_rel(tts, TB, P.ttl_ms) : req_time(tts, P.ttl_ms);
            };
            if (tp) take(tid);
            uint32_t in_use = n_tail;
            uint32_t round = 2;
            while (in_use > kWideSolo) {
                const uint32_t tag = (round << 12) | (4095u - tlid);
                Slot nr = Slot{0.0, 0};
                if (tp) {
                    nr = row[tkl];
                    bool m;
                    trep = tb_step_ft(nr, WIDE_FT_GET(tkl, nr), tpm, trq, P, m);
                    if (m) atomicMax(&own[tkl], tag);
                }
                __syncthreads();
                if (tp) {
                    const uint32_t o = own[tkl];
                    if ((o >> 12) != round || o < tag) {
                        tp = false;
                    } else if (o == tag) {
                        row[tkl] = nr;
                        WIDE_FT_SET(tkl, trq.new_t);
                        atomicOr(&dirty[tkl >> 5], 1u << (tkl & 31));
                        tp = false;
                    }
                    if (!tp) put_reply(res, tpos, trep, narrow);
                }
                ++round;
                const uint64_t bal = __ballot(tp);
                if ((tid & 63) == 0) wsum[tid >> 6] = (uint32_t)__popcll(bal);
                __syncthreads();
                uint32_t off = 0, left = 0;
#pragma unroll
                for (int w = 0; w < kWideBlock / 64; ++w) {
                    const uint32_t cw = wsum[w];
                    off += (w < (tid >> 6)) ? cw : 0u;
                    left += cw;
                }
                if (left == 0) {
                    in_use = 0;
                    break;
                }
                if ((left + 63) / 64 < (in_use + 63) / 64) {
                    if (tp) {
                        const uint32_t at = off + (uint32_t)__popcll(bal & lanemask_lt());
                        t_kl_lid[at] = tkl | (tlid << 16);
                        t_pm[at] = tpm;
                        t_ts[at] = tts;
                        t_pos[at] = tpos;
                    }
                    __syncthreads();
                    tp = (uint32_t)tid < left;
                    if (tp) take(tid);
                    in_use = left;
                }
            }
#if TBE_WIDE_SOLO
            if (in_use != 0) {
                if (tid < 64) {
                    for (;; ++round) {
                        const uint32_t tag = (round << 12) | (4095u - tlid);
                        Slot nr = Slot{0.0, 0};
                        if (tp) {
                            nr = row[tkl];
                            bool m;
                            trep = tb_step_ft(nr, WIDE_FT_GET(tkl, nr), tpm, trq, P, m);
                            if (m) atomicMax(&own[tkl], tag);
                        }
                        __builtin_amdgcn_fence(__ATOMIC_ACQ_REL, "wavefront");
                        __builtin_amdgcn_wave_barrier();
                        if (tp) {
                            const uint32_t o = own[tkl];
                            if ((o >> 12) != round || o < tag) {
                                tp = false;
                            } else if (o == tag) {
                                row[tkl] = nr;
                                WIDE_FT_SET(tkl, trq.new_t);
                                atomicOr(&dirty[tkl >> 5], 1u << (tkl & 31));
                                tp = false;
                            }
                            if (!tp) put_reply(res, tpos, trep, narrow);
                        }
                        if (!__any(tp)) break;
                        __builtin_amdgcn_fence(__ATOMIC_ACQ_REL, "wavefront");
                        __builtin_amdgcn_wave_barrier();
                    }
                }
                __syncthreads();
            }
#endif
        } else if (n_tail != 0) {
            uint32_t round = 2;
#pragma unroll
            for (int r = 0; r < kWidePer; ++r) {
                const uint32_t bit = 1u << r;
                const uint32_t tag_lo = 4095u - (uint32_t)(r * kWideBlock + tid);
                if (!__syncthreads_or(pend & bit)) continue;
                for (;; ++round) {
                    const uint32_t tag = (round << 12) | tag_lo;
                    Slot nr = Slot{0.0, 0};
                    if (pend & bit) {
                        nr = row[kl[r]];
                        bool m;
                        const ReqTime rqr = PACKED ? req_time_rel(tsv[r], TB, P.ttl_ms) : req_time(tsv[r], P.ttl_ms);
                        rep[r] = tb_step_ft(nr, WIDE_FT_GET(kl[r], nr), pm[r], rqr, P, m);
                        if (m) atomicMax(&own[kl[r]], tag);
                    }
                    __syncthreads();
                    if (pend & bit) {
                        const uint32_t o = own[kl[r]];
                        if ((o >> 12) != round || o < tag) {
                            pend &= ~bit;
                        } else if (o == tag) {
                            row[kl[r]] = nr;
                            WIDE_FT_SET(kl[r], rq[r].new_t);
                            atomicOr(&dirty[kl[r] >> 5], 1u << (kl[r] & 31));
                            pend &= ~bit;
                        }
                    }
                    if (!__syncthreads_or(pend & bit)) {
                        ++round;
                        break;
                    }
                }
            }
        }
#pragma unroll
        for (int r = 0; r < kWidePer; ++r) {
            const uint32_t q = c + r * kWideBlock + tid;
            if (q < e && (keep & (1u << r))) put_reply(res, pos[r], rep[r], narrow);
        }
    }
    __syncthreads();
    for (uint32_t j = tid; j < nrows; j += kWideBlock)
        if (row_line_dirty(dirty, j)) ST_S(rows + j, row[j]);
    if (count_hot) {
        for (uint32_t j = tid; j < nrows; j += kWideBlock) {
            if (hcnt[j] >= kHotMin) {
                const uint32_t at = atomicAdd(&hot_next->n_cand, 1u);
                if (at < kHotCandMax) hot_next->cand[at] = ((uint64_t)hcnt[j] << 32) | (uint32_t)(row0 + j);
            }
        }
    }
#if TBE_FOLD_PREFETCH
    if (wide_min == 0xFFFFFFFFu) res[s] = pf_sink;
#endif
}

constexpr int64_t kRowWindow = (int64_t)1 << 31;

__device__ __forceinline__ double field_t(int64_t t_us, const TimeBase &B) {
    return req_time_rel(t_us == kAbsent ? absent_t(B) : t_us, B, 0).new_t;
}

constexpr int kSpBlock = 256;
constexpr int kSpWaves = kSpBlock / 64;
template <bool PACKED>
__global__ __launch_bounds__(kSpBlock) void k_fold_sparse(
    const uint32_t *__restrict__ skeys, const int32_t *__restrict__ sperm,
    const int64_t *__restrict__ sts, const uint64_t *__restrict__ srec,
    const int64_t *__restrict__ ts_orig, PackFmt F, const uint32_t *__restrict__ bstart,
    int r_bits, uint64_t n_keys, Slot *__restrict__ table, TbParams P,
    uint32_t *__restrict__ res, const uint32_t *__restrict__ err, uint32_t narrow, uint32_t wide_min,
    FoldFmt G, const uint64_t *__restrict__ rec0, uint32_t n_walk) {
    if (*err) return;
    const int lane = threadIdx.x & 63;
    const uint32_t wave = blockIdx.x * kSpWaves + (threadIdx.x >> 6);
    const uint32_t nwaves = gridDim.x * kSpWaves;
    const uint32_t rmask = (1u << r_bits) - 1u;
    const int64_t tbase = PACKED ? pack_base(ts_orig, F) : 0;
    const int64_t tbase1 = G.on ? fold_base(ts_orig, G) : 0;
    const TimeBase TB = time_base(PACKED ? rel_base(ts_orig, F) : -1, P.ttl_ms);
    const uint64_t lt = lanemask_lt();
    for (uint32_t bb0 = wave; bb0 < n_walk; bb0 += nwaves * 64u) {
        const uint32_t my_bb = bb0 + (uint32_t)lane * nwaves;
        uint32_t my_b = 0xFFFFFFFFu, my_s = 0, my_e = 0;
        if (my_bb < n_walk) {
            my_b = fold_bucket_at(G, my_bb);
            if (!G.on || my_b < G.nb) {
                my_s = bstart[my_b];
                my_e = bstart[my_b + 1];
            }
        }
        uint64_t work = __ballot(my_e > my_s && my_e - my_s < wide_min);
        while (work) {
            const int j = __ffsll((long long)work) - 1;
            work &= work - 1;
            const uint32_t b = __shfl(my_b, j, 64);
            const uint32_t s = __shfl(my_s, j, 64), e = __shfl(my_e, j, 64);
            Slot *__restrict__ rows = table + ((uint64_t)b << r_bits);
            for (uint32_t c = s; c < e; c += 64) {
                if (c != s) __builtin_amdgcn_fence(__ATOMIC_SEQ_CST, "workgroup");
                const uint32_t q = c + (uint32_t)lane;
                const bool v = q < e;
                uint32_t kl = 0, pos = q;
                int32_t pm = 0;
                int64_t tsv = 0;
                if (v) {
                    if (PACKED) {
                        fold_input(LD_F(srec + q), q, G, tbase1, rec0, ts_orig, tbase, F, rmask, kl, pm, tsv, pos);
                    } else {
                        kl = skeys[q] & rmask;
                        pm = sperm[q];
                        tsv = sts[q];
                    }
                }
                uint64_t peers = __ballot(v);
                for (int bit = 0; bit < r_bits; ++bit) {
                    const bool x = (kl >> bit) & 1u;
                    const uint64_t m = __ballot(x);
                    peers &= x ? m : ~m;
                }
                const bool leader = v && (peers & lt) == 0;
                Slot st = Slot{0.0, 0};
                if (leader) st = rows[kl];
                uint64_t todo = leader ? peers : 0ull;
                bool mod = false;
                while (__any(todo != 0ull)) {
                    const int m = todo ? __ffsll((long long)todo) - 1 : lane;
                    const int32_t pm_m = __shfl(pm, m, 64);
                    const int64_t ts_m = __shfl(tsv, m, 64);
                    const uint32_t pos_m = __shfl(pos, m, 64);
                    if (todo) {
                        const ReqTime rq = PACKED ? req_time_rel(ts_m, TB, P.ttl_ms) : req_time(ts_m, P.ttl_ms);
                        bool md;
                        const uint32_t rep = tb_step_ft(st, field_t(st.t_us, TB), pm_m, rq, P, md);
                        mod |= md;
                        put_reply(res, pos_m, rep, narrow);
                        todo &= todo - 1;
                    }
                }
                if (leader && mod) rows[kl] = st;
            }
        }
    }
}

constexpr uint32_t kRemNone = 0x3FFFFFFFu;
__device__ __forceinline__ uint32_t pack_wait(uint32_t status, bool evaluated, uint32_t rem) {
    return (status << 30) | (evaluated ? (rem & kRemNone) : kRemNone);
}
constexpr uint32_t kRemNone8 = 63u;
constexpr uint32_t kRemNone16 = 0x3FFFu;
__device__ __forceinline__ void put_wait(uint32_t *res, uint32_t q, uint32_t status, bool evaluated, uint32_t rem,
                                         uint32_t rw) {
    if (rw == 1)
        reinterpret_cast<uint8_t *>(res)[q] = (uint8_t)((status << 6) | (evaluated ? (rem & 63u) : kRemNone8));
    else if (rw == 2)
        reinterpret_cast<uint16_t *>(res)[q] =
            (uint16_t)((status << 14) | (evaluated ? (rem & kRemNone16) : kRemNone16));
    else
        res[q] = pack_wait(status, evaluated, rem);
}
__device__ __forceinline__ uint16_t wait16(uint32_t v) {
    const uint32_t rem = v & kRemNone;
    return (uint16_t)(((v >> 30) << 14) | (rem == kRemNone ? kRemNone16 : (rem & kRemNone16)));
}

template <bool FINAL, bool WAIT, int W = 4>
__global__ __launch_bounds__(kUnBlock) void k_unscatter(uint64_t n, const uint32_t *__restrict__ perm,
                                                          const uint32_t *__restrict__ res_in,
                                                          uint32_t *__restrict__ res_out,
                                                          uint8_t *__restrict__ granted,
                                                          int32_t *__restrict__ remaining,
                                                          const uint32_t *__restrict__ err = nullptr,
                                                          uint32_t *__restrict__ sticky = nullptr) {
    const int tid = threadIdx.x;
    if (sticky && blockIdx.x == 0 && tid == 0 && *err) *sticky = 1u;
    const uint32_t tile = xcd_swizzle(blockIdx.x, gridDim.x);
    const uint64_t base = (uint64_t)tile * kUnTile;
    const int nvalid = (int)min<uint64_t>(kUnTile, n - base);
    uint32_t pv[kUnItems], r[kUnItems];
#pragma unroll
    for (int it = 0; it < kUnItems; ++it) {
        const int e = it * kUnBlock + tid;
        pv[it] = (e < nvalid) ? LD_U(perm + base + e) : 0u;
    }
#pragma unroll
    for (int it = 0; it < kUnItems; ++it) {
        const int e = it * kUnBlock + tid;
        r[it] = (e < nvalid) ? (W == 1 ? (uint32_t)reinterpret_cast<const uint8_t *>(res_in)[pv[it]]
                                : W == 2 ? (uint32_t)reinterpret_cast<const uint16_t *>(res_in)[pv[it]]
                                         : res_in[pv[it]])
                             : 0u;
    }
#pragma unroll
    for (int it = 0; it < kUnItems; ++it) {
        const int e = it * kUnBlock + tid;
        if (e >= nvalid) continue;
        const uint64_t i = base + e;
        if (FINAL && WAIT && W == 1) {
            ST_U(granted + i, (uint8_t)(r[it] >> 6));
            const uint32_t rem = r[it] & 63u;
            ST_U(remaining + i, (rem == kRemNone8) ? -1 : (int32_t)rem);
        } else if (FINAL && WAIT && W == 2) {
            ST_U(granted + i, (uint8_t)(r[it] >> 14));
            const uint32_t rem = r[it] & kRemNone16;
            ST_U(remaining + i, (rem == kRemNone16) ? -1 : (int32_t)rem);
        } else if (FINAL && WAIT) {
            ST_U(granted + i, (uint8_t)(r[it] >> 30));
            const uint32_t rem = r[it] & kRemNone;
            ST_U(remaining + i, (rem == kRemNone) ? -1 : (int32_t)rem);
        } else if (FINAL && W == 1) {
            ST_U(granted + i, (uint8_t)(r[it] >> 7));
            ST_U(remaining + i, (int32_t)(r[it] & 0x7Fu));
        } else if (FINAL) {
            ST_U(granted + i, (uint8_t)(r[it] >> 31));
            ST_U(remaining + i, (int32_t)(r[it] & 0x7FFFFFFFu));
        } else if (W == 1) {
            ST_U(reinterpret_cast<uint8_t *>(res_out) + i, (uint8_t)r[it]);
        } else if (W == 2) {
            ST_U(reinterpret_cast<uint16_t *>(res_out) + i, (uint16_t)r[it]);
        } else {
            ST_U(res_out + i, r[it]);
        }
    }
}

template <int W, bool WAIT = false>
__global__ __launch_bounds__(kPartBlock) void k_unrank(uint64_t n, const uint8_t *__restrict__ digit,
                                                       const uint32_t *__restrict__ tileprefix,
                                                       const uint32_t *__restrict__ blockprefix,
                                                       const uint32_t *__restrict__ digit_total,
                                                       uint32_t tiles_per_blk, const uint32_t *__restrict__ res_in,
                                                       uint8_t *__restrict__ granted,
                                                       int32_t *__restrict__ remaining) {
    __shared__ RankLds<kPartBlock> L;
    __shared__ uint32_t goff[kDigits];
    __shared__ uint32_t wcnt[(kPartBlock / 64) * kDigits];
    const uint32_t tile = xcd_swizzle(blockIdx.x, gridDim.x);
    const uint64_t base = (uint64_t)tile * kTile;
    const int nvalid = (int)min<uint64_t>(kTile, n - base);
    uint32_t dg[kPartItems], lpos[kPartItems];
#pragma unroll
    for (int it = 0; it < kPartItems; ++it) {
        const int e = wb_elem<kPartBlock, kPartItems>(it);
        dg[it] = e < nvalid ? (uint32_t)LD_U(digit + base + e) : 0u;
    }
    tile_offsets<kPartBlock>(tile, tiles_per_blk, tileprefix, blockprefix, digit_total, goff, L.wsum);
    rank_tile_wb<kPartBlock, kPartItems>(dg, 0, nvalid, L, wcnt, lpos);
    uint32_t r[kPartItems];
#pragma unroll
    for (int it = 0; it < kPartItems; ++it) {
        const int e = wb_elem<kPartBlock, kPartItems>(it);
        const uint32_t q = goff[dg[it]] + lpos[it] - L.lstart[dg[it]];
        r[it] = e < nvalid ? (W == 1   ? (uint32_t)reinterpret_cast<const uint8_t *>(res_in)[q]
                              : W == 2 ? (uint32_t)reinterpret_cast<const uint16_t *>(res_in)[q]
                                       : res_in[q])
                           : 0u;
    }
#pragma unroll
    for (int it = 0; it < kPartItems; ++it) {
        const int e = wb_elem<kPartBlock, kPartItems>(it);
        if (e >= nvalid) continue;
        const uint64_t i = base + e;
        if (WAIT && W == 1) {
            ST_U(granted + i, (uint8_t)(r[it] >> 6));
            const uint32_t rem = r[it] & 63u;
            ST_U(remaining + i, (rem == kRemNone8) ? -1 : (int32_t)rem);
        } else if (WAIT && W == 2) {
            ST_U(granted + i, (uint8_t)(r[it] >> 14));
            const uint32_t rem = r[it] & kRemNone16;
            ST_U(remaining + i, (rem == kRemNone16) ? -1 : (int32_t)rem);
        } else if (WAIT) {
            ST_U(granted + i, (uint8_t)(r[it] >> 30));
            const uint32_t rem = r[it] & kRemNone;
            ST_U(remaining + i, (rem == kRemNone) ? -1 : (int32_t)rem);
        } else if (W == 1) {
            ST_U(granted + i, (uint8_t)(r[it] >> 7));
            ST_U(remaining + i, (int32_t)(r[it] & 0x7Fu));
        } else {
            ST_U(granted + i, (uint8_t)(r[it] >> 31));
            ST_U(remaining + i, (int32_t)(r[it] & 0x7FFFFFFFu));
        }
    }
}

constexpr int kSegBlock = kFoldBlock;
constexpr int kSegItems = 16;
constexpr uint32_t kSeg = kSegBlock * kSegItems;

struct SegSummary {
    int64_t max_ts;
    int32_t min_p;
    uint32_t pad;
};
struct SegState {
    Slot s;
    double ft;
    uint32_t pass;
    uint32_t pad;
};


__device__ __forceinline__ uint32_t seg_run(const uint32_t *segbase, uint32_t j) {
    uint32_t lo = 0, hi = kHotKeysMax;
    while (hi - lo > 1) {
        const uint32_t mid = (lo + hi) >> 1;
        if (segbase[mid] <= j) lo = mid;
        else hi = mid;
    }
    return lo;
}

template <bool SPEC>
__global__ __launch_bounds__(kSegBlock) void k_hot_summary(
    const uint64_t *__restrict__ srec, const int64_t *__restrict__ ts_orig, PackFmt F,
    const uint32_t *__restrict__ bstart, uint32_t nb, uint32_t *segbase,
    SegSummary *__restrict__ summ, const uint32_t *__restrict__ err, FoldFmt G, const uint64_t *__restrict__ rec0,
    const HotSet *__restrict__ hot = nullptr, const Slot *__restrict__ table = nullptr, TbParams P = TbParams{},
    uint32_t *__restrict__ res = nullptr, uint32_t narrow = 0, uint32_t plan = 0) {
    __shared__ int64_t wts[kSegBlock / 64];
    __shared__ int32_t wp[kSegBlock / 64];
    __shared__ uint32_t pass_s0;
    __shared__ uint32_t sb[kHotKeysMax + 1];
    __shared__ uint32_t sbw[kSegBlock / 64];
    if (*err) return;
    const int tid = threadIdx.x, lane = tid & 63, w = tid >> 6;
    if (plan) {
        static_assert(kHotKeysMax == 2 * kSegBlock, "two runs per thread");
        const uint32_t cnt = hot->count;
        uint32_t ns[2];
#pragma unroll
        for (int u = 0; u < 2; ++u) {
            const uint32_t h = 2 * tid + u;
            ns[u] = h < cnt ? (bstart[nb + h + 1] - bstart[nb + h] + kSeg - 1) / kSeg : 0u;
        }
        uint32_t all;
        const uint32_t pre = block_excl_scan<kSegBlock>(ns[0] + ns[1], sbw, &all);
        sb[2 * tid] = pre;
        sb[2 * tid + 1] = pre + ns[0];
        if (tid == 0) sb[kHotKeysMax] = all;
        __syncthreads();
        if (blockIdx.x == 0) {
            for (uint32_t j = tid; j <= kHotKeysMax; j += kSegBlock) segbase[j] = sb[j];
        }
        segbase = sb;
    }
    const uint32_t total = segbase[kHotKeysMax];
    const int64_t tbase = pack_base(ts_orig, F);
    const int64_t tbase1 = G.on ? fold_base(ts_orig, G) : 0;
    const TimeBase TB = time_base(rel_base(ts_orig, F), P.ttl_ms);
    for (uint32_t j = blockIdx.x; j < total; j += gridDim.x) {
        const uint32_t h = seg_run(segbase, j);
        const uint32_t a = bstart[nb + h] + (j - segbase[h]) * kSeg;
        const uint32_t b = min(a + kSeg, bstart[nb + h + 1]);
        int64_t mx = INT64_MIN;
        int32_t mn = INT32_MAX;
// ... 1459 lines not shown
    if (at >= capacity) return;
    const uint64_t base = (uint64_t)blockIdx.x * kLiveTile;
    const int lane = threadIdx.x & 63, w = threadIdx.x >> 6;
    Slot s[kLiveItems];
    bool live[kLiveItems];
    uint32_t rank[kLiveItems];
#pragma unroll
    for (int k = 0; k < kLiveItems; ++k) {
        const uint64_t i = base + (uint64_t)k * kBlock + threadIdx.x;
        live[k] = false;
        if (i < count) {
            s[k] = slot_load_nt(&table[first + i]);
            live[k] = row_live(s[k].t_us, exp_lt);
        }
        const uint64_t bal = __ballot(live[k]);
        rank[k] = (uint32_t)__popcll(bal & lanemask_lt());
        if (lane == 0) cnt[k * kWaves + w] = (uint32_t)__popcll(bal);
    }
    __syncthreads();
    uint32_t run = 0;
#pragma unroll
    for (int k = 0; k < kLiveItems; ++k) {
#pragma unroll
        for (int w2 = 0; w2 < kWaves; ++w2) {
            if (w2 == w && live[k]) {
                const uint64_t pos = at + run + rank[k];
                if (pos < capacity) {
                    ids[pos] = first + base + (uint64_t)k * kBlock + threadIdx.x;
                    v[pos] = s[k].v;
                    t_us[pos] = s[k].t_us;
                }
            }
            run += cnt[k * kWaves + w2];
        }
    }
}

__global__ void k_rows_check(const uint64_t *__restrict__ ids, const int64_t *__restrict__ t_us, uint64_t n,
                             uint64_t n_keys, uint32_t *__restrict__ bad) {
    const uint64_t stride = (uint64_t)gridDim.x * blockDim.x;
    for (uint64_t i = (uint64_t)blockIdx.x * blockDim.x + threadIdx.x; i < n; i += stride) {
        const int64_t t = t_us[i];
        if (ids[i] >= n_keys || (t < 0 && t != kAbsent)) *bad = 1u;
    }
}

__global__ void k_rows_write(Slot *__restrict__ table, const uint64_t *__restrict__ ids, const double *__restrict__ v,
                             const int64_t *__restrict__ t_us, uint64_t n, double cap,
                             const uint32_t *__restrict__ bad, uint32_t *__restrict__ sticky) {
    if (*bad) {
        if (blockIdx.x == 0 && threadIdx.x == 0) *sticky = 1u;
        return;
    }
    const uint64_t stride = (uint64_t)gridDim.x * blockDim.x;
    for (uint64_t i = (uint64_t)blockIdx.x * blockDim.x + threadIdx.x; i < n; i += stride) {
        const int64_t t = t_us[i];
        table[ids[i]] = t == kAbsent ? Slot{cap, kAbsent} : Slot{v[i], t};
    }
}

enum Stage { ST_HIST = 0, ST_COLSCAN, ST_SCATTER, ST_BOUNDS, ST_FOLD, ST_UNSCATTER, ST_HOT, ST_COUNT };

struct PassBufs {
    uint64_t *rec = nullptr;
    uint32_t *keys = nullptr;
    int32_t *permits = nullptr;
    int64_t *ts = nullptr;
    uint32_t *idx = nullptr;
    uint32_t *perm = nullptr;
    uint32_t *tileprefix = nullptr;
    uint32_t *blockprefix = nullptr;
    uint32_t *digit_total = nullptr;
};

struct Workspace {
    uint64_t cap_n = 0;
    std::vector<PassBufs> pass;
    uint32_t *blocksum = nullptr;
    uint32_t *res[2] = {nullptr, nullptr};
    uint32_t *bstart = nullptr;
    uint32_t *bcount = nullptr;
    uint32_t *dlist = nullptr;
    unsigned long long *bsflags = nullptr;
    uint32_t bs_tag = 0;
    bool bs_fresh = false;
    uint8_t *dig0 = nullptr;
    uint8_t *dig1 = nullptr;
    int64_t *ts0 = nullptr;
    uint32_t *err = nullptr;
    hipEvent_t hot_done = nullptr;
    bool hot_pending = false;
    uint32_t *segbase = nullptr;
    SegSummary *summ = nullptr;
    SegState *sst = nullptr;
    hipEvent_t done = nullptr;
    bool used = false;
};

inline int ceil_log2(uint64_t x) {
    int b = 0;
    while ((1ull << b) < x) ++b;
    return b;
}

}

struct tbe_engine {
    tbe_config cfg{};
    int device = 0;
    hipStream_t stream = nullptr;
    bool own_stream = false;
    TbParams params{};
    int r_bits = 0;
    uint32_t nbuckets = 0;
    int passes = 0;
    bool packed = false;
    bool narrow = false;
    bool medium = false;
    uint32_t wait_rw() const { return narrow ? 1u : (medium ? 2u : 0u); }
    PackFmt pf{};
    bool foldrec = false;
    bool unrank = false;
    bool dig1 = false;
    bool n0 = false;
    uint32_t hot_cap = 0;
    uint32_t nb_total = 0;
    HotSet *hot[3] = {nullptr, nullptr, nullptr};
    uint64_t nbatch = 0;
    Slot *table = nullptr;
    QParams qp{};
    uint64_t *qhdr = nullptr;
    bool qh32 = false;
    uint64_t *ring = nullptr;
    uint64_t queued_total = 0;
    bool queued_exact = true;
    bool ev_pending = false;
    unsigned long long *qcount = nullptr;
    uint32_t *ev_cause = nullptr;
    int64_t *ev_id = nullptr;
    uint64_t ev_cap = 0;
    uint64_t *log_keyseq = nullptr;
    int64_t *log_id = nullptr;
    int32_t *log_rem = nullptr;
    uint64_t log_cap = 0;
    uint32_t *counters = nullptr;
    AParams ap{};
    ALocal *alocal = nullptr;
    AClient *aclient = nullptr;
    bool aclient_lazy = false;
    double *gv = nullptr, *gp = nullptr;
    int64_t *gt = nullptr;
    int32_t *acounts = nullptr;
    int wait_mode = 1;
    QTick qtick{-1, nullptr, nullptr, nullptr, nullptr, 0};
    std::vector<std::pair<uint64_t, int64_t>> evicted;
    std::vector<std::tuple<uint64_t, int64_t, int32_t>> drained;

    Workspace ws[2];
    int ws_cur = 0;
    bool pipeline = false;
    hipStream_t pstream = nullptr;
    hipStream_t hstream = nullptr;
    hipEvent_t ev_in = nullptr, ev_part = nullptr, ev_out = nullptr, ev_hot = nullptr;
    uint32_t *sticky = nullptr;
    uint32_t *last_err = nullptr;
    unsigned long long *live_tiles = nullptr;
    uint32_t *rows_bad = nullptr;
    hipStream_t cin = nullptr, cout = nullptr;
    hipStream_t cin2 = nullptr;
    std::vector<hipEvent_t> ev_chunk2;
    std::vector<hipEvent_t> ev_chunk;
    uint64_t stage_cap = 0;
    uint64_t *d_keys = nullptr;
    int32_t *d_permits = nullptr;
    int64_t *d_ts = nullptr;
    uint8_t *d_granted = nullptr;
    int32_t *d_remaining = nullptr;

    bool timing = false;
    uint32_t timing_mask = 0;
    std::vector<hipEvent_t> ev_pool;
    size_t ev_used = 0;
    std::vector<std::pair<int, size_t>> ev_marks;
    int open_stage = -1;
    std::string last_error = "ok";
};

template <typename F>
static void with_qhdr(tbe_engine *e, F &&f) {
    if (e->qh32) f(reinterpret_cast<uint32_t *>(e->qhdr));
    else f(e->qhdr);
}

namespace {

tbe_status fail(tbe_engine *e, tbe_status st, const char *fmt, ...) {
    char buf[512];
    va_list ap;
    va_start(ap, fmt);
    vsnprintf(buf, sizeof buf, fmt, ap);
    va_end(ap);
    if (e) e->last_error = buf;
    return st;
}

#define HIP_TRY(e, expr)                                                                    \
    do {                                                                                    \
        hipError_t _rc = (expr);                                                            \
        if (_rc != hipSuccess)                                                              \
            return fail((e), _rc == hipErrorOutOfMemory ? TBE_ENOMEM : TBE_EDEVICE,         \
                        "%s failed: %s", #expr, hipGetErrorString(_rc));                    \
    } while (0)

template <typename T>
void dfree(T *&p) {
    if (p) (void)hipFree(p);
    p = nullptr;
}

void free_workspace(Workspace &w) {
    if (w.used && w.done) (void)hipEventSynchronize(w.done);
    if (w.hot_pending && w.hot_done) (void)hipEventSynchronize(w.hot_done);
    w.hot_pending = false;
    for (auto &pb : w.pass) {
        dfree(pb.rec);
        dfree(pb.keys);
        dfree(pb.permits);
        dfree(pb.ts);
        dfree(pb.idx);
        dfree(pb.perm);
        dfree(pb.tileprefix);
        dfree(pb.blockprefix);
        dfree(pb.digit_total);
    }
    w.pass.clear();
    dfree(w.blocksum);
    dfree(w.summ);
    dfree(w.sst);
    dfree(w.segbase);
    dfree(w.res[0]);
    dfree(w.res[1]);
    dfree(w.bstart);
    dfree(w.bcount);
    w.err = nullptr;
    w.dlist = nullptr;
    dfree(w.bsflags);
    dfree(w.dig0);
    dfree(w.dig1);
    dfree(w.ts0);
    w.cap_n = 0;
    w.used = false;
}

void free_staging(tbe_engine *e) {
    dfree(e->d_keys);
    dfree(e->d_permits);
    dfree(e->d_ts);
    dfree(e->d_granted);
    dfree(e->d_remaining);
    e->stage_cap = 0;
}

void tiles_for(uint64_t n, uint32_t &ntiles, uint32_t &nblk, uint32_t &tpb) {
    ntiles = (uint32_t)((n + kTile - 1) / kTile);
    tpb = (ntiles + kMaxHistBlocks - 1) / kMaxHistBlocks;
    if (tpb == 0) tpb = 1;
    nblk = (ntiles + tpb - 1) / tpb;
}

tbe_status ensure_workspace(tbe_engine *e, Workspace &w, uint64_t n) {
    if (n <= w.cap_n) return TBE_OK;
    free_workspace(w);
    uint64_t cap = std::max<uint64_t>(n, 1u << 16);
    uint32_t ntiles, nblk, tpb;
    tiles_for(cap, ntiles, nblk, tpb);
    w.pass.resize(e->passes);
    for (auto &pb : w.pass) {
        if (e->packed) {
            HIP_TRY(e, hipMalloc(&pb.rec, cap * sizeof(uint64_t)));
        } else {
            HIP_TRY(e, hipMalloc(&pb.keys, cap * sizeof(uint32_t)));
            HIP_TRY(e, hipMalloc(&pb.permits, cap * sizeof(int32_t)));
            HIP_TRY(e, hipMalloc(&pb.ts, cap * sizeof(int64_t)));
        }
        HIP_TRY(e, hipMalloc(&pb.perm, cap * sizeof(uint32_t)));
        if (e->cfg.kind != TBE_KIND_TOKEN_BUCKET) HIP_TRY(e, hipMalloc(&pb.idx, cap * sizeof(uint32_t)));
        HIP_TRY(e, hipMalloc(&pb.tileprefix, (uint64_t)ntiles * kDigits * sizeof(uint32_t)));
        HIP_TRY(e, hipMalloc(&pb.blockprefix, (uint64_t)kMaxHistBlocks * kDigits * sizeof(uint32_t)));
        HIP_TRY(e, hipMalloc(&pb.digit_total, kDigits * sizeof(uint32_t)));
    }
    HIP_TRY(e, hipMalloc(&w.blocksum, (uint64_t)kMaxHistBlocks * kDigits * sizeof(uint32_t)));
    if (e->hot_cap) {
        const uint64_t segs = cap / kSeg + kHotKeysMax + 1;
        HIP_TRY(e, hipMalloc(&w.summ, segs * sizeof(SegSummary)));
        HIP_TRY(e, hipMalloc(&w.sst, segs * sizeof(SegState)));
        HIP_TRY(e, hipMalloc(&w.segbase, (kHotKeysMax + 1) * sizeof(uint32_t)));
    }
    HIP_TRY(e, hipMalloc(&w.res[0], cap * sizeof(uint32_t)));
    HIP_TRY(e, hipMalloc(&w.res[1], cap * sizeof(uint32_t)));
    HIP_TRY(e, hipMalloc(&w.bstart, ((uint64_t)e->nb_total + 1) * sizeof(uint32_t)));
    HIP_TRY(e, hipMalloc(&w.bcount, ((uint64_t)e->nb_total + 2 + e->nbuckets) * sizeof(uint32_t)));
    w.err = w.bcount + e->nb_total;
    w.dlist = w.bcount + e->nb_total + 1;
    HIP_TRY(e, hipMalloc(&w.bsflags, kBsMaxBlocks * sizeof(unsigned long long)));
    w.bs_fresh = true;
    w.bs_tag = 0;
    if (e->unrank) HIP_TRY(e, hipMalloc(&w.dig0, cap));
    if (e->dig1) HIP_TRY(e, hipMalloc(&w.dig1, cap));
    if (e->n0 && e->cfg.kind != TBE_KIND_APPROXIMATE) HIP_TRY(e, hipMalloc(&w.ts0, cap * sizeof(int64_t)));
    w.cap_n = cap;
    return TBE_OK;
}

tbe_status ensure_host_staging(tbe_engine *e, uint64_t n) {
    if (n <= e->stage_cap) return TBE_OK;
    free_staging(e);
    const uint64_t cap = std::max<uint64_t>(n, 1u << 16);
    HIP_TRY(e, hipMalloc(&e->d_keys, cap * sizeof(uint64_t)));
    HIP_TRY(e, hipMalloc(&e->d_permits, cap * sizeof(int32_t)));
    HIP_TRY(e, hipMalloc(&e->d_ts, cap * sizeof(int64_t)));
    HIP_TRY(e, hipMalloc(&e->d_granted, cap * sizeof(uint8_t)));
    HIP_TRY(e, hipMalloc(&e->d_remaining, cap * sizeof(int32_t)));
    e->stage_cap = cap;
    return TBE_OK;
}

hipEvent_t next_event(tbe_engine *e) {
    if (e->ev_used == e->ev_pool.size()) {
        hipEvent_t ev = nullptr;
        if (hipEventCreate(&ev) != hipSuccess) return nullptr;
        e->ev_pool.push_back(ev);
    }
    return e->ev_pool[e->ev_used++];
}
inline void stage_begin(tbe_engine *e, int s, hipStream_t st) {
    if (!e->timing || !((e->timing_mask >> s) & 1u)) return;
    const size_t idx = e->ev_used;
    hipEvent_t a = next_event(e), b = next_event(e);
    if (!a || !b) return;
    (void)hipEventRecord(a, st);
    e->ev_marks.emplace_back(s, idx);
    (void)b;
}
inline void stage_end(tbe_engine *e, int s, hipStream_t st) {
    if (!e->timing || e->ev_marks.empty() || e->ev_marks.back().first != s) return;
    (void)hipEventRecord(e->ev_pool[e->ev_marks.back().second + 1], st);
}

#ifndef TBE_SPARSE_GATE_SHIFT
#define TBE_SPARSE_GATE_SHIFT 3
#endif
uint32_t fold_wide_min(const tbe_engine *e, uint64_t n) {
    const uint32_t R = 1u << e->r_bits;
    const uint32_t all = std::max(1u, R >> kWideMinShift);
    if (n >= (uint64_t)e->nbuckets * std::max(1u, R >> TBE_SPARSE_GATE_SHIFT)) return all;
    return std::max(all, R >> 3);
}

#ifndef TBE_HOT_SPARSE_MIN_LOG2
#define TBE_HOT_SPARSE_MIN_LOG2 20
#endif
inline uint32_t hot_reserve_host(uint32_t cap) { return std::min(32u, cap / 4u); }

FoldFmt batch_fold_fmt(const tbe_engine *e, uint64_t n) {
    FoldFmt G{};
    if (!e->foldrec) return G;
    const bool approx = e->cfg.kind == TBE_KIND_APPROXIMATE;
    const int pw = std::max(1, ceil_log2(n));
    const int tw = 64 - e->r_bits - e->pf.pb - 1 - pw;
    if (tw >= (approx ? 1 : 8)) {
        G.on = 1;
        G.n0 = (e->n0 && !(approx && e->wait_mode)) ? 1 : 0;
        G.rb = e->r_bits;
        G.pb = e->pf.pb;
        G.pw = pw;
        G.tw = tw;
        G.nb = e->nbuckets;
        G.region_bits = (uint32_t)(kDigitBits * (e->passes - 1));
        G.n_hi = (uint32_t)(((uint64_t)e->nbuckets + (1ull << G.region_bits) - 1) >> G.region_bits);
    }
    return G;
}

tbe_status run_batch(tbe_engine *e, const uint64_t *keys, const int32_t *permits,
                     const int64_t *ts, uint64_t n, uint8_t *granted, int32_t *remaining,
                     hipStream_t caller, int64_t id_base = 0, hipEvent_t in_ready = nullptr,
                     hipStream_t out_stream = nullptr, uint32_t ai_base = 0) {
    const bool approx = e->cfg.kind == TBE_KIND_APPROXIMATE;
    const bool wait = e->cfg.kind != TBE_KIND_TOKEN_BUCKET;
    if (n == 0) return TBE_OK;
    if (n >= (1ull << 32)) return fail(e, TBE_EINVAL, "batch of %llu requests exceeds 2^32-1",
                                       (unsigned long long)n);
    if (e->packed && !approx && !ts) return fail(e, TBE_EINVAL, "null timestamps");
    const bool pipe = e->pipeline;
    Workspace &w = e->ws[pipe ? e->ws_cur : 0];
    tbe_status rc = ensure_workspace(e, w, n);
    if (rc != TBE_OK) return rc;
    uint32_t ntiles, nblk, tpb;
    tiles_for(n, ntiles, nblk, tpb);
    hipStream_t sf = caller ? caller : e->stream, sp = sf;
    if (pipe) {
        sf = e->stream;
        sp = e->pstream;
        if (in_ready) {
            HIP_TRY(e, hipStreamWaitEvent(sp, in_ready, 0));
        } else if (caller) {
            HIP_TRY(e, hipEventRecord(e->ev_in, caller));
            HIP_TRY(e, hipStreamWaitEvent(sp, e->ev_in, 0));
        }
        if (w.used) HIP_TRY(e, hipStreamWaitEvent(sp, w.done, 0));
        if (w.hot_pending) HIP_TRY(e, hipStreamWaitEvent(sp, w.hot_done, 0));
    } else if (in_ready) {
        HIP_TRY(e, hipStreamWaitEvent(sf, in_ready, 0));
    }
    HIP_TRY(e, hipMemsetAsync(w.bcount, 0, ((uint64_t)e->nb_total + 2) * sizeof(uint32_t), sp));
    if (w.bs_fresh) {
        HIP_TRY(e, hipMemsetAsync(w.bsflags, 0, kBsMaxBlocks * sizeof(unsigned long long), sp));
        w.bs_fresh = false;
    }

    const uint64_t kmask = e->packed ? e->pf.kmask : ~0ull;
    const FoldFmt G = batch_fold_fmt(e, n);
    PackFmt pf = e->pf;
    pf.n0 = G.n0;
    const uint64_t *rec0 = G.on ? (G.n0 ? reinterpret_cast<const uint64_t *>(w.ts0) : w.pass[e->passes - 2].rec)
                                : nullptr;
    const bool unrank = e->unrank;
    const unsigned fold_grid = G.on ? (unsigned)((1ull << G.region_bits) * G.n_hi) : e->nbuckets;
    const uint32_t tb_wmin = (!approx && !wait) ? fold_wide_min(e, n) : 1u;
    const bool sparse_tb = tb_wmin > 1u;
    const bool hot_on = e->hot_cap && !(sparse_tb && n < (1ull << TBE_HOT_SPARSE_MIN_LOG2));
    HotSet *hot = hot_on ? e->hot[e->nbatch % 3] : nullptr;
    HotSet *hot_next = hot_on ? e->hot[(e->nbatch + 2) % 3] : nullptr;
    if (hot && n >= kHotSampleMin) k_hot_sample<<<1, 1024, 0, sp>>>(keys, n, e->cfg.n_keys, hot, e->hot_cap);
    for (int p = 0; p < e->passes; ++p) {
        const int shift = e->r_bits + kDigitBits * p;
        PassBufs &out = w.pass[p];
        stage_begin(e, ST_HIST, sp);
        uint32_t *bc = (p == e->passes - 1) ? w.bcount : nullptr;
        const int lowbits = kDigitBits * p;
        uint8_t *dig = (p == 0 && unrank) ? w.dig0 : nullptr;
        uint8_t *dnext = (p == 0 && e->dig1) ? w.dig1 : nullptr;
        if (p == 0 && hot)
            k_hist<uint64_t, true><<<nblk, kHBlock, 0, sp>>>(keys, n, shift, tpb, ntiles, out.tileprefix,
                                                             w.blocksum, e->cfg.n_keys, w.err, 1, kmask,
                                                             hot, e->nbuckets, e->r_bits, bc, lowbits,
                                                             e->nb_total, dig);
        else if (p == 0)
            k_hist<uint64_t><<<nblk, kHBlock, 0, sp>>>(keys, n, shift, tpb, ntiles, out.tileprefix,
                                                       w.blocksum, e->cfg.n_keys, w.err, 1, kmask,
                                                       nullptr, e->nbuckets, e->r_bits, bc, lowbits,
                                                       e->nb_total, dig);
        else if (e->dig1 && p == 1)
            k_hist_dig<<<nblk, kHBlock, 0, sp>>>(w.dig1, n, tpb, ntiles, out.tileprefix, w.blocksum,
                                                 w.pass[0].digit_total, bc, e->nb_total);
        else if (e->packed)
            k_hist<uint64_t><<<nblk, kHBlock, 0, sp>>>(w.pass[p - 1].rec, n, shift, tpb, ntiles,
                                                       out.tileprefix, w.blocksum, e->cfg.n_keys,
                                                       w.err, 0, kmask, nullptr, e->nbuckets,
                                                       e->r_bits, bc, lowbits, e->nb_total);
        else
            k_hist<uint32_t><<<nblk, kHBlock, 0, sp>>>(w.pass[p - 1].keys, n, shift, tpb, ntiles,
                                                       out.tileprefix, w.blocksum, e->cfg.n_keys,
                                                       w.err, 0, kmask, nullptr, e->nbuckets,
                                                       e->r_bits, bc, lowbits, e->nb_total);
        stage_end(e, ST_HIST, sp);
        stage_begin(e, ST_COLSCAN, sp);
        k_colscan<<<kDigits, kBlock, 0, sp>>>(w.blocksum, nblk, out.blockprefix, out.digit_total);
        stage_end(e, ST_COLSCAN, sp);
        stage_begin(e, ST_SCATTER, sp);
#define LAUNCH_LAST_FAM(IDXK, FAMK, iin_, iout_)                                                               \
    k_scatter_rec<false, false, IDXK, false, true, FAMK><<<ntiles, kPartBlock, 0, sp>>>(                       \
        nullptr, nullptr, ts, w.pass[p - 1].rec, n, shift, pf, out.tileprefix, out.blockprefix,                \
        out.digit_total, tpb, out.rec, nullptr, w.err, nullptr, 0, 0, iin_, iout_, G, nullptr, w.dig1, nullptr, \
        pass1_codec(pf, G, true))
#define LAUNCH_LAST(IDXK, iin_, iout_)                                                     \
    do {                                                                                   \
        if (TBE_PASS1_CODEC && G.n0 && pass1_codec_ok(pf, G))                              \
            LAUNCH_LAST_FAM(IDXK, 1, iin_, iout_);                                         \
        else if (TBE_PASS1_CODEC && !G.n0)                                                 \
            LAUNCH_LAST_FAM(IDXK, 0, iin_, iout_);                                         \
        else                                                                               \
            LAUNCH_LAST_FAM(IDXK, -1, iin_, iout_);                                        \
    } while (0)
        if (e->packed && approx && p == 0)
            k_scatter_rec<true, false, false, true><<<ntiles, kPartBlock, 0, sp>>>(
                keys, permits, nullptr, nullptr, n, shift, pf, out.tileprefix, out.blockprefix,
                out.digit_total, tpb, out.rec, unrank ? nullptr : out.perm, w.err, nullptr, 0, 0, nullptr,
                nullptr, FoldFmt{}, dnext);
        else if (e->packed && approx && G.on && p == e->passes - 1)
            k_scatter_rec<false, false, false, false, true><<<ntiles, kPartBlock, 0, sp>>>(
                nullptr, nullptr, nullptr, w.pass[p - 1].rec, n, shift, pf, out.tileprefix,
                out.blockprefix, out.digit_total, tpb, out.rec, nullptr, w.err, nullptr, 0, 0, nullptr,
                nullptr, G, nullptr, w.dig1);
        else if (e->packed && approx)
            k_scatter_rec<false><<<ntiles, kPartBlock, 0, sp>>>(
                nullptr, nullptr, nullptr, w.pass[p - 1].rec, n, shift, e->pf, out.tileprefix,
                out.blockprefix, out.digit_total, tpb, out.rec, out.perm, w.err);
        else if (e->packed && wait && p == 0)
            k_scatter_rec<true, false, true><<<ntiles, kPartBlock, 0, sp>>>(
                keys, permits, ts, nullptr, n, shift, pf, out.tileprefix, out.blockprefix,
                out.digit_total, tpb, out.rec, unrank ? nullptr : out.perm, w.err, nullptr, 0, 0, nullptr, out.idx,
                FoldFmt{}, dnext, nullptr, w.ts0);
        else if (e->packed && wait && G.on && p == e->passes - 1)
            LAUNCH_LAST_FAM(true, -1, w.pass[p - 1].idx, out.idx);
        else if (e->packed && wait)
            k_scatter_rec<false, false, true><<<ntiles, kPartBlock, 0, sp>>>(
                nullptr, nullptr, nullptr, w.pass[p - 1].rec, n, shift, e->pf, out.tileprefix,
                out.blockprefix, out.digit_total, tpb, out.rec, out.perm, w.err, nullptr, 0, 0,
                w.pass[p - 1].idx, out.idx);
        else if (e->packed && p == 0 && hot)
            k_scatter_rec<true, true><<<ntiles, kPartBlock, 0, sp>>>(
                keys, permits, ts, nullptr, n, shift, pf, out.tileprefix, out.blockprefix,
                out.digit_total, tpb, out.rec, unrank ? nullptr : out.perm, w.err, hot, e->nbuckets, e->r_bits,
                nullptr, nullptr, FoldFmt{}, dnext, nullptr, w.ts0);
        else if (e->packed && p == 0)
            k_scatter_rec<true><<<ntiles, kPartBlock, 0, sp>>>(
                keys, permits, ts, nullptr, n, shift, pf, out.tileprefix, out.blockprefix,
                out.digit_total, tpb, out.rec, unrank ? nullptr : out.perm, w.err, nullptr, 0, 0, nullptr,
                nullptr, FoldFmt{}, dnext, nullptr, w.ts0);
        else if (e->packed && G.on && p == e->passes - 1)
            LAUNCH_LAST(false, nullptr, nullptr);
        else if (e->packed)
            k_scatter_rec<false><<<ntiles, kPartBlock, 0, sp>>>(
                nullptr, nullptr, nullptr, w.pass[p - 1].rec, n, shift, e->pf, out.tileprefix,
                out.blockprefix, out.digit_total, tpb, out.rec, out.perm, w.err);
        else if (approx && p == 0)
            k_scatter<uint64_t, true, false><<<ntiles, kPartBlock, 0, sp>>>(
                keys, permits, nullptr, nullptr, n, shift, out.tileprefix, out.blockprefix,
                out.digit_total, tpb, out.keys, out.permits, nullptr, out.idx, out.perm, w.err, 1);
        else if (approx)
            k_scatter<uint32_t, true, false><<<ntiles, kPartBlock, 0, sp>>>(
                w.pass[p - 1].keys, w.pass[p - 1].permits, nullptr, w.pass[p - 1].idx, n, shift,
                out.tileprefix, out.blockprefix, out.digit_total, tpb, out.keys, out.permits, nullptr,
                out.idx, out.perm, w.err, 0);
        else if (p == 0 && !wait)
            k_scatter<uint64_t, false><<<ntiles, kPartBlock, 0, sp>>>(
                keys, permits, ts, nullptr, n, shift, out.tileprefix, out.blockprefix,
                out.digit_total, tpb, out.keys, out.permits, out.ts, nullptr, out.perm, w.err, 1);
        else if (p == 0)
            k_scatter<uint64_t, true><<<ntiles, kPartBlock, 0, sp>>>(
                keys, permits, ts, nullptr, n, shift, out.tileprefix, out.blockprefix,
                out.digit_total, tpb, out.keys, out.permits, out.ts, out.idx, out.perm, w.err, 1);
        else if (!wait)
            k_scatter<uint32_t, false><<<ntiles, kPartBlock, 0, sp>>>(
                w.pass[p - 1].keys, w.pass[p - 1].permits, w.pass[p - 1].ts, nullptr, n, shift,
                out.tileprefix, out.blockprefix, out.digit_total, tpb, out.keys, out.permits,
                out.ts, nullptr, out.perm, w.err, 0);
        else
            k_scatter<uint32_t, true><<<ntiles, kPartBlock, 0, sp>>>(
                w.pass[p - 1].keys, w.pass[p - 1].permits, w.pass[p - 1].ts, w.pass[p - 1].idx,
                n, shift, out.tileprefix, out.blockprefix, out.digit_total, tpb, out.keys,
                out.permits, out.ts, out.idx, out.perm, w.err, 0);
        stage_end(e, ST_SCATTER, sp);
    }
    const PassBufs &sorted = w.pass[e->passes - 1];
    stage_begin(e, ST_BOUNDS, sp);
    const uint32_t bs_blocks = (e->nb_total + kBsTile - 1) / kBsTile;
    if (TBE_BSCAN_LB && bs_blocks <= kBsMaxBlocks) {
        if (++w.bs_tag == 0) {
            HIP_TRY(e, hipMemsetAsync(w.bsflags, 0, kBsMaxBlocks * sizeof(unsigned long long), sp));
            w.bs_tag = 1;
        }
        k_bscan_lb<<<bs_blocks, 1024, 0, sp>>>(w.bcount, e->nb_total, w.bstart, w.bsflags, w.bs_tag,
                                               e->nbuckets, tb_wmin, sparse_tb ? w.dlist : nullptr);
    }
    else if (sparse_tb)
        k_bscan<<<1, 1024, 0, sp>>>(w.bcount, e->nb_total, w.bstart, e->nbuckets, tb_wmin, w.dlist);
    else
        k_bscan<<<1, 1024, 0, sp>>>(w.bcount, e->nb_total, w.bstart);
    stage_end(e, ST_BOUNDS, sp);
    if (pipe) {
        HIP_TRY(e, hipEventRecord(e->ev_part, sp));
        HIP_TRY(e, hipStreamWaitEvent(sf, e->ev_part, 0));
    }
#define LAUNCH_WIDE_FAM(FAMK, grid_, dlist_)                                                              \
    k_fold_wide<true, FAMK><<<grid_, kWideBlock, 0, sf>>>(                                                \
        nullptr, nullptr, nullptr, sorted.rec, ts, e->pf, w.bstart, e->r_bits, e->cfg.n_keys, e->table,   \
        e->params, w.res[0], w.err, hot_next, e->narrow ? 1u : 0u, tb_wmin, G, rec0, dlist_)
#define LAUNCH_WIDE(grid_, dlist_)                      \
    do {                                                \
        if (!TBE_FOLD_FAM)                              \
            LAUNCH_WIDE_FAM(-1, grid_, dlist_);         \
        else if (!G.on)                                 \
            LAUNCH_WIDE_FAM(0, grid_, dlist_);          \
        else if (G.n0)                                  \
            LAUNCH_WIDE_FAM(1, grid_, dlist_);          \
        else                                            \
            LAUNCH_WIDE_FAM(2, grid_, dlist_);          \
    } while (0)
    stage_begin(e, ST_FOLD, sf);
    if (approx) {
        AParams a = e->ap;
        a.id_base = id_base;
        a.wait = e->wait_mode;
        a.ai_base = ai_base;
        if (e->packed)
            k_fold_a<true><<<fold_grid, kFoldBlock, 0, sf>>>(
                nullptr, nullptr, nullptr, sorted.rec, e->pf, w.bstart, e->r_bits, e->cfg.n_keys, e->alocal,
                e->ring, a, w.res[0], e->ev_cause, e->ev_id, e->counters,
                (uint32_t)std::min<uint64_t>(e->ev_cap, 0xFFFFFFFFu), w.err, e->wait_rw(), G, rec0);
        else
            k_fold_a<false><<<e->nbuckets, kFoldBlock, 0, sf>>>(
                sorted.keys, sorted.permits, sorted.idx, nullptr, e->pf, w.bstart, e->r_bits, e->cfg.n_keys,
                e->alocal, e->ring, a, w.res[0], e->ev_cause, e->ev_id, e->counters,
                (uint32_t)std::min<uint64_t>(e->ev_cap, 0xFFFFFFFFu), w.err, e->wait_rw(), G, rec0);
    } else if (wait) {
        QParams q = e->qp;
        q.id_base = id_base;
        q.wait = e->wait_mode;
        q.ai_base = ai_base;
        with_qhdr(e, [&](auto *qh) {
            using HW = std::remove_pointer_t<decltype(qh)>;
            if (e->packed)
                k_fold_q<true, HW><<<fold_grid, kQBlock, 0, sf>>>(
                    nullptr, nullptr, nullptr, sorted.idx, sorted.rec, ts, e->pf, w.bstart, e->r_bits,
                    e->cfg.n_keys, e->table, qh, e->ring, e->params, q, w.res[0], e->ev_cause, e->ev_id,
                    e->counters, (uint32_t)std::min<uint64_t>(e->ev_cap, 0xFFFFFFFFu), w.err, e->wait_rw(),
                    e->qtick, G, rec0);
            else
                k_fold_q<false, HW><<<e->nbuckets, kQBlock, 0, sf>>>(
                    sorted.keys, sorted.permits, sorted.ts, sorted.idx, nullptr, nullptr, e->pf, w.bstart,
                    e->r_bits, e->cfg.n_keys, e->table, qh, e->ring, e->params, q, w.res[0], e->ev_cause,
                    e->ev_id, e->counters, (uint32_t)std::min<uint64_t>(e->ev_cap, 0xFFFFFFFFu), w.err,
                    e->wait_rw(), e->qtick, G, rec0);
        });
    } else if (sparse_tb) {
        const unsigned dgrid = (unsigned)std::min<uint64_t>(e->nbuckets, n / tb_wmin + 1);
        const uint32_t walk = e->packed ? fold_grid : e->nbuckets;
        const unsigned sgrid = (unsigned)std::min<uint64_t>((walk + kSpWaves - 1) / kSpWaves, 2048);
        if (e->packed) {
            LAUNCH_WIDE(dgrid, w.dlist);
            k_fold_sparse<true><<<sgrid, kSpBlock, 0, sf>>>(
                nullptr, nullptr, nullptr, sorted.rec, ts, e->pf, w.bstart, e->r_bits, e->cfg.n_keys,
                e->table, e->params, w.res[0], w.err, e->narrow ? 1u : 0u, tb_wmin, G, rec0, walk);
        } else {
            k_fold_wide<false><<<dgrid, kWideBlock, 0, sf>>>(
                sorted.keys, sorted.permits, sorted.ts, nullptr, nullptr, e->pf, w.bstart, e->r_bits,
                e->cfg.n_keys, e->table, e->params, w.res[0], w.err, nullptr, 0u, tb_wmin, G, rec0, w.dlist);
            k_fold_sparse<false><<<sgrid, kSpBlock, 0, sf>>>(
                sorted.keys, sorted.permits, sorted.ts, nullptr, nullptr, e->pf, w.bstart, e->r_bits,
                e->cfg.n_keys, e->table, e->params, w.res[0], w.err, 0u, tb_wmin, G, rec0, walk);
        }
    } else if (e->packed) {
        LAUNCH_WIDE(fold_grid, nullptr);
    } else {
        k_fold_wide<false><<<e->nbuckets, kWideBlock, 0, sf>>>(
            sorted.keys, sorted.permits, sorted.ts, nullptr, nullptr, e->pf, w.bstart, e->r_bits,
            e->cfg.n_keys, e->table, e->params, w.res[0], w.err, nullptr, 0u, tb_wmin, G, rec0);
    }
    stage_end(e, ST_FOLD, sf);
    if (hot) {
        stage_begin(e, ST_HOT, sf);
        const unsigned sgrid = (unsigned)std::min<uint64_t>(1024, n / kSeg + e->hot_cap);
        k_hot_summary<true><<<sgrid, kSegBlock, 0, sf>>>(sorted.rec, ts, e->pf, w.bstart, e->nbuckets,
                                                             w.segbase, w.summ, w.err, G, rec0, hot, e->table,
                                                             e->params, w.res[0], e->narrow ? 1u : 0u, 1u);
        k_hot_chain<<<e->hot_cap, kSegBlock, 0, sf>>>(sorted.rec, ts, e->pf, w.bstart, e->nbuckets, hot,
                                                      hot_next, w.segbase, w.summ, w.sst, e->table,
                                                      e->params, w.res[0], w.err, e->narrow ? 1u : 0u, G, rec0,
                                                      1u);
        k_hot_replies<<<sgrid, kSegBlock, 0, sf>>>(sorted.rec, ts, e->pf, w.bstart, e->nbuckets,
                                                   w.segbase, w.sst, e->params, w.res[0], w.err, e->narrow ? 1u : 0u,
                                                   G, rec0);
        if (pipe) {
            HIP_TRY(e, hipEventRecord(e->ev_hot, sf));
            HIP_TRY(e, hipStreamWaitEvent(e->hstream, e->ev_hot, 0));
            k_hot_update<<<1, 1024, 0, e->hstream>>>(hot_next, e->hot_cap - hot_reserve_host(e->hot_cap), w.err);
            HIP_TRY(e, hipEventRecord(w.hot_done, e->hstream));
            w.hot_pending = true;
        } else {
            k_hot_update<<<1, 1024, 0, sf>>>(hot_next, e->hot_cap - hot_reserve_host(e->hot_cap), w.err);
        }
        stage_end(e, ST_HOT, sf);
    }
    stage_begin(e, ST_UNSCATTER, sf);
    const unsigned untiles = (unsigned)((n + kUnTile - 1) / kUnTile);
    int cur = 0;
    for (int p = e->passes - (G.on ? 2 : 1); p >= 1; --p) {
        if (e->narrow && !approx)
            k_unscatter<false, false, 1><<<untiles, kUnBlock, 0, sf>>>(n, w.pass[p].perm, w.res[cur],
                                                                   w.res[cur ^ 1], nullptr, nullptr);
        else if (e->medium)
            k_unscatter<false, false, 2><<<untiles, kUnBlock, 0, sf>>>(n, w.pass[p].perm, w.res[cur],
                                                                   w.res[cur ^ 1], nullptr, nullptr);
        else
            k_unscatter<false, false><<<untiles, kUnBlock, 0, sf>>>(n, w.pass[p].perm, w.res[cur],
                                                                    w.res[cur ^ 1], nullptr, nullptr);
        cur ^= 1;
    }
#define TBE_UNRANK(...)                                                                             \
    __VA_ARGS__<<<ntiles, kPartBlock, 0, sf>>>(n, w.dig0, w.pass[0].tileprefix, w.pass[0].blockprefix, \
                                               w.pass[0].digit_total, tpb, w.res[cur], granted, remaining)
    if (unrank && !wait && e->narrow)
        TBE_UNRANK(k_unrank<1>);
    else if (unrank && !wait)
        TBE_UNRANK(k_unrank<4>);
    else if (unrank && e->narrow)
        TBE_UNRANK(k_unrank<1, true>);
    else if (unrank && e->medium)
        TBE_UNRANK(k_unrank<2, true>);
    else if (unrank)
        TBE_UNRANK(k_unrank<4, true>);
#undef TBE_UNRANK
    else if (e->narrow && !wait && !approx)
        k_unscatter<true, false, 1><<<untiles, kUnBlock, 0, sf>>>(n, w.pass[0].perm, w.res[cur],
                                                                  nullptr, granted, remaining,
            w.err, e->sticky);
    else if (wait && e->narrow)
        k_unscatter<true, true, 1><<<untiles, kUnBlock, 0, sf>>>(n, w.pass[0].perm, w.res[cur],
                                                                 nullptr, granted, remaining,
            w.err, e->sticky);
    else if (wait && e->medium)
        k_unscatter<true, true, 2><<<untiles, kUnBlock, 0, sf>>>(n, w.pass[0].perm, w.res[cur],
                                                                 nullptr, granted, remaining,
            w.err, e->sticky);
    else if (wait)
        k_unscatter<true, true><<<untiles, kUnBlock, 0, sf>>>(n, w.pass[0].perm, w.res[cur],
                                                              nullptr, granted, remaining,
            w.err, e->sticky);
    else
        k_unscatter<true, false><<<untiles, kUnBlock, 0, sf>>>(n, w.pass[0].perm, w.res[cur],
                                                               nullptr, granted, remaining,
            w.err, e->sticky);
    stage_end(e, ST_UNSCATTER, sf);
    if (unrank) k_sticky<<<1, 64, 0, sf>>>(w.err, e->sticky);
    HIP_TRY(e, hipGetLastError());
    if (pipe) {
        HIP_TRY(e, hipEventRecord(w.done, sf));
        w.used = true;
        hipStream_t outs = out_stream ? out_stream : caller;
        if (outs && outs != sf) {
            HIP_TRY(e, hipEventRecord(e->ev_out, sf));
            HIP_TRY(e, hipStreamWaitEvent(outs, e->ev_out, 0));
        }
        e->ws_cur ^= 1;
    } else if (out_stream && out_stream != sf) {
        HIP_TRY(e, hipEventRecord(e->ev_out, sf));
        HIP_TRY(e, hipStreamWaitEvent(out_stream, e->ev_out, 0));
    }
    e->last_err = w.err;
    ++e->nbatch;
    return TBE_OK;
}

}

template <typename T>
hipError_t dalloc(T **p, size_t bytes) {
    return hipMalloc(reinterpret_cast<void **>(p), bytes);
}

extern "C" {

double tbe_fill_rate(int32_t tokens_per_period, int64_t replenishment_period_ticks) {
    const double total_seconds = (double)replenishment_period_ticks / 10000000.0;
    return (double)tokens_per_period / total_seconds;
}

static thread_local std::string g_create_error = "no error";

static tbe_status create_fail(tbe_status st, const char *msg) {
    g_create_error = msg;
    return st;
}

tbe_status tbe_create(const tbe_config *config, tbe_engine **out_engine) {
    if (!out_engine) return create_fail(TBE_EINVAL, "out_engine is NULL");
    *out_engine = nullptr;
    constexpr size_t kConfigV1 = offsetof(tbe_config, zero_wait_slots);
    if (!config || config->struct_size < kConfigV1)
        return create_fail(TBE_EINVAL, "config is NULL or struct_size too small");
    tbe_config c_in;
    std::memset(&c_in, 0, sizeof c_in);
    std::memcpy(&c_in, config, std::min<size_t>(config->struct_size, sizeof c_in));
    const tbe_config &c = c_in;
    if (c.kind != TBE_KIND_TOKEN_BUCKET && c.kind != TBE_KIND_QUEUEING &&
        c.kind != TBE_KIND_APPROXIMATE)
        return create_fail(TBE_EINVAL, "unknown kind");
    if (c.kind != TBE_KIND_TOKEN_BUCKET) {
        if (c.queue_limit < 0 || c.queue_limit > 0xFFFF)
            return create_fail(TBE_EINVAL, "QueueLimit must lie in [0, 65535]");
        if (c.queue_order != 0 && c.queue_order != 1)
            return create_fail(TBE_EINVAL, "QueueProcessingOrder must be OldestFirst (0) or NewestFirst (1)");
        if (c.token_limit >= (int32_t)kRemNone)
            return create_fail(TBE_EINVAL, "TokenLimit must be < 2^30 - 1 for queueing limiters");
        if (c.zero_wait_slots < 0 || (c.kind == TBE_KIND_QUEUEING && c.zero_wait_slots != 0) ||
            std::max(1, c.queue_limit) + c.zero_wait_slots > 0xFFFF)
            return create_fail(TBE_EINVAL, "zero_wait_slots must be >= 0 (approximate kind only) with "
                                           "max(1, QueueLimit) + zero_wait_slots <= 65535");
    }
    if (c.n_keys == 0 || c.n_keys > (1ull << 32))
        return create_fail(TBE_EINVAL, "n_keys must lie in [1, 2^32]");
    if (c.token_limit <= 0 || c.tokens_per_period <= 0)
        return create_fail(TBE_EINVAL, "Both TokenLimit and TokensPerPeriod must be set to values greater than 0.");
    if (c.replenishment_period_ticks <= 0)
        return create_fail(TBE_EINVAL, "ReplenishmentPeriod must be greater than TimeSpan.Zero");
    const double rate = tbe_fill_rate(c.tokens_per_period, c.replenishment_period_ticks);
    if (!std::isfinite(rate) || !(rate > 0.0)) return create_fail(TBE_EINVAL, "fill rate is not finite and positive");

    tbe_engine *e = new (std::nothrow) tbe_engine();
    if (!e) return create_fail(TBE_ENOMEM, "host allocation failed");
    e->cfg = c;
    e->params.cap = (double)c.token_limit;
    e->params.rate = rate;
    {
        double q = (double)c.token_limit / rate;
        q = (1.0 > q) ? 1.0 : q;
        q = (31536000.0 < q) ? 31536000.0 : q;
        e->params.ttl_ms = (int64_t)std::ceil(q) * 1000;
    }
    const int kb = ceil_log2(c.n_keys);
    e->r_bits = std::min(kMaxRBits, std::max(4, kb - 10));
    e->nbuckets = (uint32_t)((c.n_keys + (1ull << e->r_bits) - 1) >> e->r_bits);
    const int bbits = ceil_log2(e->nbuckets);
    e->passes = std::max(1, (bbits + kDigitBits - 1) / kDigitBits);
    e->timing = (c.flags & (TBE_FLAG_STAGE_TIMING | TBE_FLAG_FOLD_TIMING)) != 0;
    e->timing_mask = (c.flags & TBE_FLAG_STAGE_TIMING) ? ~0u : (1u << ST_FOLD);
    {
        int pbits = 0;
        while (pbits < 32 && ((int64_t)1 << pbits) <= (int64_t)c.token_limit + 1) ++pbits;
        auto layout = [&](uint32_t hot_cap) {
            const uint64_t span = std::max<uint64_t>(c.n_keys, ((uint64_t)e->nbuckets + hot_cap) << e->r_bits);
            const int kbits = std::max(1, ceil_log2(span));
            e->pf.kb = kbits;
            e->pf.pb = pbits;
            e->pf.kmask = (kbits >= 64) ? ~0ull : ((1ull << kbits) - 1);
            e->pf.pc_max = (c.token_limit == INT32_MAX) ? INT32_MAX : c.token_limit + 1;
            e->pf.wb = 64 - kbits - pbits - 1;
            return e->pf.wb >= 32 && kbits <= 32 && (c.flags & TBE_FLAG_NO_PACK) == 0;
        };
        uint32_t hot_cap = 0;
        if ((c.flags & TBE_FLAG_NO_HOT) == 0 && c.kind == TBE_KIND_TOKEN_BUCKET) {
            const uint64_t room = (1ull << (kDigitBits * e->passes)) - e->nbuckets;
            hot_cap = (uint32_t)std::min<uint64_t>(kHotKeysMax, room);
            if (hot_cap < 16) hot_cap = 0;
        }
        e->packed = hot_cap && layout(hot_cap);
        if (!e->packed) {
            hot_cap = 0;
            e->packed = layout(0);
        }
        e->hot_cap = hot_cap;
        e->nb_total = e->nbuckets + hot_cap;
        e->foldrec = e->packed && e->passes >= 2 && (c.flags & TBE_FLAG_UNSCATTER_ALL) == 0;
        e->unrank = e->packed && (c.flags & TBE_FLAG_UNSCATTER_ALL) == 0 && (c.flags & TBE_FLAG_RERANK) != 0;
        e->dig1 = e->packed && e->passes == 2 && (c.flags & TBE_FLAG_HIST_RECORDS) == 0;
        {
            const int w0 = 32 - e->r_bits - pbits - 1;
            e->n0 = TBE_NARROW0 && e->dig1 && e->foldrec &&
                    (c.kind == TBE_KIND_APPROXIMATE ? e->r_bits + pbits + 1 <= 32 : w0 >= 8);
            e->pf.n0 = 0;
            e->pf.rb = e->r_bits;
            e->pf.w0 = w0;
        }
        e->narrow = (c.flags & TBE_FLAG_NO_NARROW) == 0 &&
                    ((e->packed && c.kind == TBE_KIND_TOKEN_BUCKET && c.token_limit <= 127) ||
                     (c.kind == TBE_KIND_QUEUEING && c.token_limit <= 62));
        e->medium = (c.flags & TBE_FLAG_NO_NARROW) == 0 && !e->narrow && c.token_limit <= (int32_t)kRemNone16 - 1 &&
                    (c.kind == TBE_KIND_QUEUEING || c.kind == TBE_KIND_APPROXIMATE);
    }

    auto bail = [&](tbe_status st) {
        tbe_destroy(e);
        return create_fail(st, st == TBE_ENOMEM ? "device allocation failed" : "HIP device error");
    };
    if (c.device >= 0) {
        if (hipSetDevice(c.device) != hipSuccess) return bail(TBE_EDEVICE);
        e->device = c.device;
    } else if (hipGetDevice(&e->device) != hipSuccess) {
        return bail(TBE_EDEVICE);
    }
    e->pipeline = c.kind == TBE_KIND_TOKEN_BUCKET && (c.flags & TBE_FLAG_NO_PIPELINE) == 0;
    if (hipStreamCreateWithFlags(&e->stream, hipStreamNonBlocking) != hipSuccess)
        return bail(TBE_EDEVICE);
    e->own_stream = true;
    if (e->pipeline && hipStreamCreateWithFlags(&e->pstream, hipStreamNonBlocking) != hipSuccess)
        return bail(TBE_EDEVICE);
    if (e->pipeline && hipStreamCreateWithFlags(&e->hstream, hipStreamNonBlocking) != hipSuccess)
        return bail(TBE_EDEVICE);
    for (hipEvent_t *ev : {&e->ev_in, &e->ev_part, &e->ev_out, &e->ev_hot, &e->ws[0].done, &e->ws[1].done,
                           &e->ws[0].hot_done, &e->ws[1].hot_done})
        if (hipEventCreateWithFlags(ev, hipEventDisableTiming) != hipSuccess) return bail(TBE_EDEVICE);
    const uint64_t qhdr_n = (c.n_keys + 3) & ~3ull;
    uint64_t ring_n = 0;
    if (dalloc(&e->table, c.n_keys * sizeof(Slot)) != hipSuccess) return bail(TBE_ENOMEM);
    if (e->hot_cap)
        for (auto &hs : e->hot)
// ... 1234 lines not shown
```

Before: 43.07 billion decisions/s.

## Evaluate wide fold with 32-bit relative timestamps and magic-number bucket division

Adds a relative-time path for the wide fold kernel. A per-batch FoldRel base is computed once inside the bucket-scan kernel, and the per-request time maths (seconds conversion, TTL expiry, grant timestamp) then runs on 32-bit offsets instead of 64-bit integer division. A wave-wide ballot falls back to the generic path when any row or record lies outside the window. The change also replaces the fold bucket division with a host-verified magic multiply, switches prefetch touches to global_load_lds, and uses a custom block-OR reduction. The cost is extra code complexity and fallback branches, plus a second library build with the feature disabled.

```diff
diff --git a/__graft_entry__.py b/__graft_entry__.py
--- a/__graft_entry__.py
+++ b/__graft_entry__.py
@@ -16,6 +16,7 @@
     mod = importlib.util.module_from_spec(spec)
     spec.loader.exec_module(mod)
     mod.build_engine(verbose=True)
+    mod.build_engine(verbose=True, defines=mod.REL32_OFF_DEFINES, out=mod.REL32_OFF_LIB)
     mod.build_host(verbose=True)
     from oracle.build import build_oracle
 
diff --git a/distributedratelimiting.redis_amd/build.py b/distributedratelimiting.redis_amd/build.py
--- a/distributedratelimiting.redis_amd/build.py
+++ b/distributedratelimiting.redis_amd/build.py
@@ -8,7 +8,7 @@
 HERE = os.path.dirname(os.path.realpath(__file__))
 ROOT = os.path.dirname(HERE)
 SOURCES = [os.path.join(HERE, "csrc", n) for n in ("tbe_engine.hip", "tbe_tools.hip", "tbe_cluster.hip", "tbe_strdir.hip")]
-DEPS = SOURCES + [os.path.join(HERE, "csrc", n) for n in ("tbe_device.hpp", "tbe_codec.hpp", "tbe_numfmt.hpp", "tbe_hash.hpp")] + \
+DEPS = SOURCES + [os.path.join(HERE, "csrc", n) for n in ("tbe_device.hpp", "tbe_codec.hpp", "tbe_reltime.hpp", "tbe_numfmt.hpp", "tbe_hash.hpp")] + \
     [os.path.join(ROOT, "include", n) for n in ("tbe.h", "tbe_tools.h", "tbe_cluster.h", "tbe_strdir.h")]
 LIB = os.path.join(HERE, "libtbe.so")
 ARCH = "gfx950"
@@ -61,6 +61,9 @@
     return out
 
 
+REL32_OFF_DEFINES = ("TBE_FOLD_REL32=0",)
+REL32_OFF_LIB = os.path.join(HERE, "libtbe_rel32_off.so")
+
 HOST_SRC = os.path.join(HERE, "host", "rate_limiting.cpp")
 HOST_DEPS = [HOST_SRC, os.path.join(HERE, "host", "rate_limiting.hpp"), os.path.join(ROOT, "include", "tbe.h")]
 HOST_LIB = os.path.join(HERE, "libtbe_host.so")
diff --git a/distributedratelimiting.redis_amd/csrc/tbe_codec.hpp b/distributedratelimiting.redis_amd/csrc/tbe_codec.hpp
--- a/distributedratelimiting.redis_amd/csrc/tbe_codec.hpp
+++ b/distributedratelimiting.redis_amd/csrc/tbe_codec.hpp
@@ -33,6 +33,7 @@
     uint32_t nb;
     uint32_t region_bits;
     uint32_t n_hi;
+    uint32_t n_hi_mul;
 };
 TBE_CODEC_FN uint64_t fold_rec32(uint32_t r32, uint32_t pos, int64_t tbase0, int64_t tbase1, const PackFmt &F,
                            const FoldFmt &G) {
diff --git a/distributedratelimiting.redis_amd/csrc/tbe_device.hpp b/distributedratelimiting.redis_amd/csrc/tbe_device.hpp
--- a/distributedratelimiting.redis_amd/csrc/tbe_device.hpp
+++ b/distributedratelimiting.redis_amd/csrc/tbe_device.hpp
@@ -109,14 +109,14 @@
 #endif
 __device__ __forceinline__ int64_t absent_t(const TimeBase &B) { return TBE_ABSENT_BASE ? B.tbase : 0; }
 
-__device__ __forceinline__ uint32_t tb_step_ft(Slot &row, double ft, int32_t permits,
-                                               const ReqTime &rq, const TbParams &P, bool &modified) {
-    const bool had = row.t_us != kAbsent;
-    const bool expired = had && row.t_us < rq.exp_lt;
+__device__ __forceinline__ uint32_t tb_step_core(Slot &row, bool had, bool lapsed, double ft, int32_t permits,
+                                                 double new_t, int64_t grant_ts, const TbParams &P,
+                                                 bool &modified) {
+    const bool expired = had && lapsed;
     const bool present = had && !expired;
     const double pv = present ? row.v : P.cap;
-    const double pt = present ? ft : rq.new_t;
-    const double delta_t = lua_max(0.0, rq.new_t - pt);
+    const double pt = present ? ft : new_t;
+    const double delta_t = lua_max(0.0, new_t - pt);
     const double fill = delta_t * P.rate;
     double x = lua_max(0.0, lua_min(P.cap, pv + fill));
     const double p = (double)permits;
@@ -124,13 +124,17 @@
     if (granted) {
         x = x - p;
         row.v = x;
-        row.t_us = rq.ts;
+        row.t_us = grant_ts;
     } else if (expired) {
         row.v = P.cap;
         row.t_us = kAbsent;
     }
     modified = granted || expired;
     return (granted ? 0x80000000u : 0u) | (uint32_t)(int32_t)x;
+}
+__device__ __forceinline__ uint32_t tb_step_ft(Slot &row, double ft, int32_t permits,
+                                               const ReqTime &rq, const TbParams &P, bool &modified) {
+    return tb_step_core(row, row.t_us != kAbsent, row.t_us < rq.exp_lt, ft, permits, rq.new_t, rq.ts, P, modified);
 }
 
 __device__ __forceinline__ uint32_t tb_step(Slot &row, int32_t permits, const ReqTime &rq,
diff --git a/distributedratelimiting.redis_amd/csrc/tbe_engine.hip b/distributedratelimiting.redis_amd/csrc/tbe_engine.hip
--- a/distributedratelimiting.redis_amd/csrc/tbe_engine.hip
+++ b/distributedratelimiting.redis_amd/csrc/tbe_engine.hip
@@ -1,6 +1,7 @@
 #include <hip/hip_runtime.h>
 
 #include <algorithm>
+#include <atomic>
 #include <cmath>
 #include <cstdarg>
 #include <cstdio>
@@ -16,6 +17,7 @@
 #include "../../include/tbe.h"
 #include "tbe_device.hpp"
 #include "tbe_codec.hpp"
+#include "tbe_reltime.hpp"
 #include "tbe_numfmt.hpp"
 
 #pragma clang fp contract(off)
@@ -598,9 +600,16 @@
 }
 
 constexpr int kScanPer = 16;
+struct RelCfg {
+    int32_t tw, w0;
+    int64_t ttl_ms;
+};
 __global__ __launch_bounds__(1024) void k_bscan(const uint32_t *__restrict__ bcount, uint32_t nbt,
                                                 uint32_t *__restrict__ bstart, uint32_t nb = 0,
-                                                uint32_t wide_min = 0, uint32_t *__restrict__ dlist = nullptr) {
+                                                uint32_t wide_min = 0, uint32_t *__restrict__ dlist = nullptr,
+                                                const int64_t *__restrict__ ts = nullptr,
+                                                FoldRel *__restrict__ rel = nullptr, RelCfg rc = RelCfg{}) {
+    if (rel && threadIdx.x == 0) *rel = fold_rel_make(ts[0], rc.tw, rc.w0, rc.ttl_ms);
     __shared__ uint32_t tile[1024 * (kScanPer + 1)];
     auto pad = [](uint32_t j) { return (j / kScanPer) * (kScanPer + 1) + (j % kScanPer); };
     __shared__ uint32_t wsum[16];
@@ -670,10 +679,13 @@
                                                    uint32_t *__restrict__ bstart,
                                                    unsigned long long *__restrict__ flags, uint32_t tag,
                                                    uint32_t nb = 0, uint32_t wide_min = 0,
-                                                   uint32_t *__restrict__ dlist = nullptr) {
+                                                   uint32_t *__restrict__ dlist = nullptr,
+                                                   const int64_t *__restrict__ ts = nullptr,
+                                                   FoldRel *__restrict__ rel = nullptr, RelCfg rc = RelCfg{}) {
     __shared__ uint32_t wsum[16];
     __shared__ uint32_t excl;
     const uint32_t t = threadIdx.x, blk = blockIdx.x;
+    if (rel && blk == 0 && t == 0) *rel = fold_rel_make(ts[0], rc.tw, rc.w0, rc.ttl_ms);
     const uint32_t b0 = blk * kBsTile + t * kBsPer;
     uint32_t v[kBsPer];
 #pragma unroll
@@ -769,6 +781,9 @@
     return row | (pc << G.rb) | ((uint64_t)!fits << (G.rb + G.pb)) | ((uint64_t)pos << (G.rb + G.pb + 1)) |
            ((fits ? d : 0ull) << (G.rb + G.pb + 1 + G.pw));
 }
+#ifndef TBE_FOLD_REL32
+#define TBE_FOLD_REL32 1
+#endif
 __device__ __forceinline__ void unfold_rec(uint64_t rec, const FoldFmt &G, int64_t tbase1,
                                            const uint64_t *__restrict__ rec0, const int64_t *__restrict__ ts_orig,
                                            int64_t tbase0, const PackFmt &F, uint32_t &row, int32_t &p,
@@ -791,7 +806,11 @@
 __device__ __forceinline__ uint32_t fold_bucket_at(const FoldFmt &G, uint32_t blk) {
     if (!G.on) return blk;
     const uint32_t x = blk & 7u, s = blk >> 3;
+#if TBE_FOLD_REL32
+    const uint32_t j = fold_div(s, G.n_hi_mul), hi = s - j * G.n_hi;
+#else
     const uint32_t j = s / G.n_hi, hi = s - j * G.n_hi;
+#endif
     return (hi << G.region_bits) | (x + 8u * j);
 }
 __device__ __forceinline__ uint32_t fold_bucket(const FoldFmt &G) { return fold_bucket_at(G, blockIdx.x); }
@@ -1107,7 +1126,38 @@
 #define WIDE_FT_GET(j, srow) req_time_rel((srow).t_us == kAbsent ? absent_t(TB) : (srow).t_us, TB, 0).new_t
 #define WIDE_FT_SET(j, v) ((void)0)
 
-template <bool PACKED, int FAM = -1>
+__device__ __forceinline__ uint32_t wide_eval_generic(Slot &nr, int32_t p, uint32_t fld, uint32_t ps,
+                                                      const uint64_t *__restrict__ rec0, const FoldRel &B,
+                                                      const TbParams &P, bool &m) {
+    const int64_t ts = fld == kRelEsc ? (int64_t)rec0[ps] : rel_grant_ts(fld, B);
+    const ReqTime rq = req_time(ts, P.ttl_ms);
+    const double ft = new_t_of(nr.t_us == kAbsent ? 0 : nr.t_us);
+    return tb_step_ft(nr, ft, p, rq, P, m);
+}
+struct RelReq {
+    double new_t;
+    uint32_t K;
+};
+__device__ __forceinline__ RelReq rel_req(uint32_t fld, const FoldRel &B) {
+    return RelReq{rel_new_t(B.u0 + fld, B.sec0), rel_ms1000(B.rr0 + fld)};
+}
+__device__ __forceinline__ uint32_t wide_eval_fast(Slot &nr, uint32_t dr, int32_t p, const RelReq &q, const FoldRel &B,
+                                                   const TbParams &P, bool &m) {
+    const double ft = rel_new_t(B.usec0 + dr, B.sec0);
+    const bool lapsed = rel_expired(dr, q.K, B.ttl32);
+    return tb_step_core(nr, nr.t_us != kAbsent, lapsed, ft, p, q.new_t, 0, P, m);
+}
+__device__ __forceinline__ uint32_t wide_eval_rel(Slot &nr, int32_t p, uint32_t fld, uint32_t ps, const RelReq &q,
+                                                  const uint64_t *__restrict__ rec0, const FoldRel &B,
+                                                  const TbParams &P, bool &m) {
+    const uint64_t off = (uint64_t)nr.t_us - (uint64_t)B.tbase;
+    const bool slow = fld == kRelEsc || (nr.t_us != kAbsent && rel_row_slow(off));
+    if (__builtin_expect(!B.fast || __builtin_amdgcn_ballot_w64(slow) != 0, 0))
+        return wide_eval_generic(nr, p, fld, ps, rec0, B, P, m);
+    return wide_eval_fast(nr, (uint32_t)off, p, q, B, P, m);
+}
+
+template <bool PACKED, int FAM = -1, bool REL = false>
 __global__ __launch_bounds__(kWideBlock, TBE_WIDE_WAVES) void k_fold_wide(
     const uint32_t *__restrict__ skeys, const int32_t *__restrict__ sperm,
     const int64_t *__restrict__ sts, const uint64_t *__restrict__ srec,
@@ -1115,7 +1165,8 @@
     int r_bits, uint64_t n_keys, Slot *__restrict__ table, TbParams P,
     uint32_t *__restrict__ res, const uint32_t *__restrict__ err, HotSet *__restrict__ hot_next,
     uint32_t narrow, uint32_t wide_min, FoldFmt G, const uint64_t *__restrict__ rec0,
-    const uint32_t *__restrict__ dlist = nullptr) {
+    const uint32_t *__restrict__ dlist = nullptr, const FoldRel *__restrict__ relp = nullptr) {
+    static_assert(!REL || (PACKED && FAM == 1), "relative times: fold records over narrow pass-0 records");
     __shared__ Slot row[kMaxRows];
     __shared__ uint64_t aux[kWideTail * 2 + kWideTail / 2];
     __shared__ uint32_t wsum[kWideBlock / 64];
@@ -1154,8 +1205,9 @@
     if (e - s < wide_min) return;
     const bool dense = true;
     const int64_t tbase = (PACKED && FAM != 1) ? pack_base(ts_orig, F) : 0;
-    const int64_t tbase1 = (FAM < 0 ? G.on != 0 : FAM >= 1) ? fold_base(ts_orig, G) : 0;
-    const TimeBase TB = time_base(PACKED ? rel_base(ts_orig, F) : 0, P.ttl_ms);
+    const int64_t tbase1 = (!REL && (FAM < 0 ? G.on != 0 : FAM >= 1)) ? fold_base(ts_orig, G) : 0;
+    const TimeBase TB = REL ? TimeBase{} : time_base(PACKED ? rel_base(ts_orig, F) : 0, P.ttl_ms);
+    const FoldRel B = REL ? *relp : FoldRel{};
     const bool count_hot = hot_next != nullptr && (e - s) >= kHotMin;
 
     uint32_t kl[kWidePer];
@@ -1173,7 +1225,14 @@
             tsv[r] = 0;
             pos[r] = q;
             if (q < e) {
-                if (PACKED) {
+                if (REL) {
+                    const uint64_t rec = LD_F(srec + q);
+                    kl[r] = (uint32_t)(rec & ((1ull << G.rb) - 1));
+                    pm[r] = (int32_t)((rec >> G.rb) & ((1ull << G.pb) - 1));
+                    pos[r] = (uint32_t)((rec >> (G.rb + G.pb + 1)) & ((1ull << G.pw) - 1));
+                    const bool esc = (rec >> (G.rb + G.pb)) & 1;
+                    tsv[r] = (int64_t)(uint64_t)(esc ? kRelEsc : rel_fld((uint32_t)(rec >> (G.rb + G.pb + 1 + G.pw)), B));
+                } else if (PACKED) {
                     fold_input_fam<FAM>(LD_F(srec + q), q, G, tbase1, rec0, ts_orig, tbase, F, rmask, kl[r], pm[r],
                                         tsv[r], pos[r]);
                 } else {
@@ -1188,6 +1247,13 @@
 
 #if TBE_FOLD_PREFETCH
     uint32_t pf_sink = 0;
+    __shared__ uint32_t pf_dump[REL ? 64 : 1];
+    auto touch = [&](const void *p) {
+        if constexpr (REL)
+            __builtin_amdgcn_global_load_lds((gvoid_t *)p, (lvoid_t *)pf_dump, 4, 0, 0);
+        else
+            pf_sink = *reinterpret_cast<const uint32_t *>(p);
+    };
 #endif
     load_chunk(s);
     if (dense) slice_dma();
@@ -1216,17 +1282,19 @@
         __syncthreads();
 #if TBE_FOLD_PREFETCH
         if (c == s && e - s >= TBE_FOLD_PREFETCH_MIN) {
+            int ptid = tid;
+            if constexpr (REL) asm volatile("" : "+v"(ptid));
             const uint32_t fblk = blockIdx.x + TBE_FOLD_PREFETCH;
             const uint32_t fb = fold_bucket_at(G, fblk);
             if (fblk < gridDim.x && (!G.on || fb < G.nb)) {
                 const uint32_t fs = bstart[fb], fe = bstart[fb + 1];
                 if (fe - fs >= wide_min && fe > fs) {
-                    if (tid < (int)(kMaxRows / 8)) {
-                        const uint64_t fr = ((uint64_t)fb << r_bits) + (uint64_t)tid * 8u;
-                        if (fr < n_keys) pf_sink = reinterpret_cast<const uint32_t *>(table + fr)[0];
+                    if (ptid < (int)(kMaxRows / 8)) {
+                        const uint64_t fr = ((uint64_t)fb << r_bits) + (uint64_t)ptid * 8u;
+                        if (fr < n_keys) touch(table + fr);
                     } else if (PACKED) {
-                        const uint32_t q = fs + (uint32_t)(tid - kMaxRows / 8) * 16u;
-                        if (q < fe) pf_sink = (uint32_t)srec[q];
+                        const uint32_t q = fs + (uint32_t)(ptid - kMaxRows / 8) * 16u;
+                        if (q < fe) touch(srec + q);
                     }
                 }
             }
@@ -1240,6 +1308,40 @@
         uint32_t rep[kWidePer];
 #pragma unroll
         for (int r = 0; r < kWidePer; ++r) rep[r] = 0;
+        auto eval_req = [&](Slot &nr, int32_t p, int64_t tv, uint32_t ps, bool &m) -> uint32_t {
+            if constexpr (REL) {
+                return wide_eval_rel(nr, p, (uint32_t)tv, ps, rel_req((uint32_t)tv, B), rec0, B, P, m);
+            } else {
+                const ReqTime rqr = PACKED ? req_time_rel(tv, TB, P.ttl_ms) : req_time(tv, P.ttl_ms);
+                return tb_step_ft(nr, WIDE_FT_GET(0, nr), p, rqr, P, m);
+            }
+        };
+        auto block_or = [&](bool p) -> bool {
+            if constexpr (REL) {
+                const bool w = __any(p);
+                if ((tid & 63) == 0) wsum[tid >> 6] = w ? 1u : 0u;
+                __syncthreads();
+                uint32_t a = 0;
+#pragma unroll
+                for (int v = 0; v < kWideBlock / 64; ++v) a |= wsum[v];
+                __syncthreads();
+                return a != 0;
+            } else {
+                return __syncthreads_or(p) != 0;
+            }
+        };
+        auto commit_row = [&](const Slot &nr, uint32_t rp, int64_t tv, uint32_t ps) -> Slot {
+            if constexpr (REL) {
+                const uint32_t f = (uint32_t)tv;
+                int64_t t = rel_grant_ts(f, B);
+                if (__builtin_expect(__builtin_amdgcn_ballot_w64(f == kRelEsc) != 0, 0)) {
+                    if (f == kRelEsc) t = (int64_t)rec0[ps];
+                }
+                return Slot{nr.v, (rp >> 31) ? t : kAbsent};
+            } else {
+                return nr;
+            }
+        };
         auto eval_slots = [&](uint32_t round, Slot (&nrow)[kWidePer]) {
 #pragma unroll
             for (int r = 0; r < kWidePer; ++r) {
@@ -1247,8 +1349,7 @@
                 if (pend & (1u << r)) {
                     nrow[r] = row[kl[r]];
                     bool m;
-                    const ReqTime rqr = PACKED ? req_time_rel(tsv[r], TB, P.ttl_ms) : req_time(tsv[r], P.ttl_ms);
-                    rep[r] = tb_step_ft(nrow[r], WIDE_FT_GET(kl[r], nrow[r]), pm[r], rqr, P, m);
+                    rep[r] = eval_req(nrow[r], pm[r], tsv[r], pos[r], m);
                     if (m) atomicMax(&own[kl[r]], (round << 12) | (4095u - (uint32_t)(r * kWideBlock + tid)));
                 }
             }
@@ -1262,7 +1363,7 @@
                 if ((o >> 12) != round || o < tag) {
                     pend &= ~(1u << r);
                 } else if (o == tag) {
-                    row[kl[r]] = nrow[r];
+                    row[kl[r]] = commit_row(nrow[r], rep[r], tsv[r], pos[r]);
                     WIDE_FT_SET(kl[r], rq[r].new_t);
                     atomicOr(&dirty[kl[r] >> 5], 1u << (kl[r] & 31));
                     pend &= ~(1u << r);
@@ -1301,13 +1402,24 @@
             int32_t tpm = 0;
             int64_t tts = 0;
             ReqTime trq{0.0, 0, 0};
+            RelReq trel{0.0, 0u};
             auto take = [&](uint32_t at) {
                 tkl = t_kl_lid[at] & 0xFFFFu;
                 tlid = t_kl_lid[at] >> 16;
                 tpm = t_pm[at];
                 tts = t_ts[at];
                 tpos = t_pos[at];
-                trq = PACKED ? req_time_rel(tts, TB, P.ttl_ms) : req_time(tts, P.ttl_ms);
+                if constexpr (REL)
+                    trel = rel_req((uint32_t)tts, B);
+                else
+                    trq = PACKED ? req_time_rel(tts, TB, P.ttl_ms) : req_time(tts, P.ttl_ms);
+            };
+            auto eval_tail = [&](Slot &nr, bool &m) -> uint32_t {
+                if constexpr (REL) {
+                    return wide_eval_rel(nr, tpm, (uint32_t)tts, tpos, trel, rec0, B, P, m);
+                } else {
+                    return tb_step_ft(nr, WIDE_FT_GET(tkl, nr), tpm, trq, P, m);
+                }
             };
             if (tp) take(tid);
             uint32_t in_use = n_tail;
@@ -1318,7 +1430,7 @@
                 if (tp) {
                     nr = row[tkl];
                     bool m;
-                    trep = tb_step_ft(nr, WIDE_FT_GET(tkl, nr), tpm, trq, P, m);
+                    trep = eval_tail(nr, m);
                     if (m) atomicMax(&own[tkl], tag);
                 }
                 __syncthreads();
@@ -1327,7 +1439,7 @@
                     if ((o >> 12) != round || o < tag) {
                         tp = false;
                     } else if (o == tag) {
-                        row[tkl] = nr;
+                        row[tkl] = commit_row(nr, trep, tts, tpos);
                         WIDE_FT_SET(tkl, trq.new_t);
                         atomicOr(&dirty[tkl >> 5], 1u << (tkl & 31));
                         tp = false;
@@ -1372,7 +1484,7 @@
                         if (tp) {
                             nr = row[tkl];
                             bool m;
-                            trep = tb_step_ft(nr, WIDE_FT_GET(tkl, nr), tpm, trq, P, m);
+                            trep = eval_tail(nr, m);
                             if (m) atomicMax(&own[tkl], tag);
                         }
                         __builtin_amdgcn_fence(__ATOMIC_ACQ_REL, "wavefront");
@@ -1382,7 +1494,7 @@
                             if ((o >> 12) != round || o < tag) {
                                 tp = false;
                             } else if (o == tag) {
-                                row[tkl] = nr;
+                                row[tkl] = commit_row(nr, trep, tts, tpos);
                                 WIDE_FT_SET(tkl, trq.new_t);
                                 atomicOr(&dirty[tkl >> 5], 1u << (tkl & 31));
                                 tp = false;
@@ -1403,15 +1515,14 @@
             for (int r = 0; r < kWidePer; ++r) {
                 const uint32_t bit = 1u << r;
                 const uint32_t tag_lo = 4095u - (uint32_t)(r * kWideBlock + tid);
-                if (!__syncthreads_or(pend & bit)) continue;
+                if (!block_or((pend & bit) != 0)) continue;
                 for (;; ++round) {
                     const uint32_t tag = (round << 12) | tag_lo;
                     Slot nr = Slot{0.0, 0};
                     if (pend & bit) {
                         nr = row[kl[r]];
                         bool m;
-                        const ReqTime rqr = PACKED ? req_time_rel(tsv[r], TB, P.ttl_ms) : req_time(tsv[r], P.ttl_ms);
-                        rep[r] = tb_step_ft(nr, WIDE_FT_GET(kl[r], nr), pm[r], rqr, P, m);
+                        rep[r] = eval_req(nr, pm[r], tsv[r], pos[r], m);
                         if (m) atomicMax(&own[kl[r]], tag);
                     }
                     __syncthreads();
@@ -1420,13 +1531,13 @@
                         if ((o >> 12) != round || o < tag) {
                             pend &= ~bit;
                         } else if (o == tag) {
-                            row[kl[r]] = nr;
+                            row[kl[r]] = commit_row(nr, rep[r], tsv[r], pos[r]);
                             WIDE_FT_SET(kl[r], rq[r].new_t);
                             atomicOr(&dirty[kl[r] >> 5], 1u << (kl[r] & 31));
                             pend &= ~bit;
                         }
                     }
-                    if (!__syncthreads_or(pend & bit)) {
+                    if (!block_or((pend & bit) != 0)) {
                         ++round;
                         break;
                     }
@@ -1451,7 +1562,7 @@
         }
     }
 #if TBE_FOLD_PREFETCH
-    if (wide_min == 0xFFFFFFFFu) res[s] = pf_sink;
+    if (!REL && wide_min == 0xFFFFFFFFu) res[s] = pf_sink;
 #endif
 }
 
@@ -3517,7 +3628,7 @@
     HIP_TRY(e, hipMalloc(&w.bcount, ((uint64_t)e->nb_total + 2 + e->nbuckets) * sizeof(uint32_t)));
     w.err = w.bcount + e->nb_total;
     w.dlist = w.bcount + e->nb_total + 1;
-    HIP_TRY(e, hipMalloc(&w.bsflags, kBsMaxBlocks * sizeof(unsigned long long)));
+    HIP_TRY(e, hipMalloc(&w.bsflags, kBsMaxBlocks * sizeof(unsigned long long) + sizeof(FoldRel)));
     w.bs_fresh = true;
     w.bs_tag = 0;
     if (e->unrank) HIP_TRY(e, hipMalloc(&w.dig0, cap));
@@ -3593,6 +3704,18 @@
         G.nb = e->nbuckets;
         G.region_bits = (uint32_t)(kDigitBits * (e->passes - 1));
         G.n_hi = (uint32_t)(((uint64_t)e->nbuckets + (1ull << G.region_bits) - 1) >> G.region_bits);
+#if TBE_FOLD_REL32
+        const uint32_t grid = (uint32_t)((1ull << G.region_bits) * G.n_hi);
+        G.n_hi_mul = fold_div_magic(G.n_hi);
+        static std::atomic<uint64_t> checked{0};
+        const uint64_t id = ((uint64_t)G.n_hi << 32) | grid;
+        if (checked.load(std::memory_order_relaxed) != id) {
+            bool ok = fold_div_ok(G.n_hi, grid) && grid <= (1u << 24);
+            for (uint32_t s = 0; ok && s <= (grid >> 3); ++s) ok = fold_div(s, G.n_hi_mul) == s / G.n_hi;
+            if (!ok) return FoldFmt{};
+            checked.store(id, std::memory_order_relaxed);
+        }
+#endif
     }
     return G;
 }
@@ -3770,6 +3893,10 @@
         stage_end(e, ST_SCATTER, sp);
     }
     const PassBufs &sorted = w.pass[e->passes - 1];
+    const bool use_rel = TBE_FOLD_REL32 && TBE_FOLD_FAM && !approx && !wait && e->packed && G.on && G.n0 &&
+                         pass1_codec_ok(pf, G) && rel_fmt_ok(G.tw, pf.w0);
+    FoldRel *relp = use_rel ? reinterpret_cast<FoldRel *>(w.bsflags + kBsMaxBlocks) : nullptr;
+    const RelCfg relcfg = use_rel ? RelCfg{G.tw, pf.w0, e->params.ttl_ms} : RelCfg{};
     stage_begin(e, ST_BOUNDS, sp);
     const uint32_t bs_blocks = (e->nb_total + kBsTile - 1) / kBsTile;
     if (TBE_BSCAN_LB && bs_blocks <= kBsMaxBlocks) {
@@ -3778,12 +3905,12 @@
             w.bs_tag = 1;
         }
         k_bscan_lb<<<bs_blocks, 1024, 0, sp>>>(w.bcount, e->nb_total, w.bstart, w.bsflags, w.bs_tag,
-                                               e->nbuckets, tb_wmin, sparse_tb ? w.dlist : nullptr);
+                                               e->nbuckets, tb_wmin, sparse_tb ? w.dlist : nullptr, ts, relp, relcfg);
     }
     else if (sparse_tb)
-        k_bscan<<<1, 1024, 0, sp>>>(w.bcount, e->nb_total, w.bstart, e->nbuckets, tb_wmin, w.dlist);
+        k_bscan<<<1, 1024, 0, sp>>>(w.bcount, e->nb_total, w.bstart, e->nbuckets, tb_wmin, w.dlist, ts, relp, relcfg);
     else
-        k_bscan<<<1, 1024, 0, sp>>>(w.bcount, e->nb_total, w.bstart);
+        k_bscan<<<1, 1024, 0, sp>>>(w.bcount, e->nb_total, w.bstart, 0u, 0u, nullptr, ts, relp, relcfg);
     stage_end(e, ST_BOUNDS, sp);
     if (pipe) {
         HIP_TRY(e, hipEventRecord(e->ev_part, sp));
@@ -3799,6 +3926,10 @@
             LAUNCH_WIDE_FAM(-1, grid_, dlist_);         \
         else if (!G.on)                                 \
             LAUNCH_WIDE_FAM(0, grid_, dlist_);          \
+        else if (use_rel)                               \
+            k_fold_wide<true, 1, true><<<grid_, kWideBlock, 0, sf>>>(                                          \
+                nullptr, nullptr, nullptr, sorted.rec, ts, e->pf, w.bstart, e->r_bits, e->cfg.n_keys, e->table, \
+                e->params, w.res[0], w.err, hot_next, e->narrow ? 1u : 0u, tb_wmin, G, rec0, dlist_, relp);    \
         else if (G.n0)                                  \
             LAUNCH_WIDE_FAM(1, grid_, dlist_);          \
         else                                            \
diff --git a/distributedratelimiting.redis_amd/csrc/tbe_reltime.hpp b/distributedratelimiting.redis_amd/csrc/tbe_reltime.hpp
--- /dev/null
+++ b/distributedratelimiting.redis_amd/csrc/tbe_reltime.hpp
@@ -0,0 +1,95 @@
+#pragma once
+#include <cstdint>
+
+#if defined(__HIPCC__)
+#define TBE_REL_FN __host__ __device__ __forceinline__
+#else
+#define TBE_REL_FN inline
+#endif
+
+constexpr int64_t kRelAbsent = INT64_MIN;
+constexpr uint64_t kRelWindow = 0xFFFFFFFFull - 1000000ull;
+constexpr uint32_t kRelEsc = 0xFFFFFFFFu;
+
+
+struct FoldRel {
+    int64_t tbase;
+    int64_t e0;
+    int64_t tbase0;
+    uint32_t sec0;
+    uint32_t usec0;
+    uint32_t r0;
+    uint32_t ok;
+    uint32_t u0;
+    uint32_t rr0;
+    uint32_t ttl32;
+    uint32_t fast;
+    uint32_t fsub;
+    uint32_t pad_;
+};
+
+TBE_REL_FN uint64_t rel_fld_max(int32_t w0) { return (1ull << w0) - 1ull; }
+TBE_REL_FN bool rel_fmt_ok(int32_t tw, int32_t w0) {
+    return w0 >= 1 && w0 <= 30 && tw >= w0 && tw <= 63 && rel_fld_max(w0) < kRelEsc;
+}
+
+TBE_REL_FN FoldRel fold_rel_make(int64_t ts0, int32_t tw, int32_t w0, int64_t ttl_ms) {
+    const uint64_t fld_max = rel_fld_max(w0);
+    FoldRel B{};
+    const int64_t rb = ts0 - ((int64_t)1 << 31);
+    B.tbase = rb > 0 ? rb : 0;
+    B.tbase0 = ts0 - ((int64_t)1 << (w0 - 1));
+    B.fsub = (uint32_t)((1ull << (tw - 1)) - (1ull << (w0 - 1)));
+    if (B.tbase >= 0) {
+        const int64_t sec0 = B.tbase / 1000000;
+        if (sec0 <= (int64_t)0xFFFFFFFFll - 10000) {
+            B.sec0 = (uint32_t)sec0;
+            B.usec0 = (uint32_t)(B.tbase - sec0 * 1000000);
+            B.r0 = (uint32_t)(B.tbase % 1000);
+            B.e0 = (B.tbase / 1000 - ttl_ms) * 1000;
+            B.ok = 1;
+        }
+    }
+    const int64_t dC = B.tbase0 - B.tbase;
+    const bool ttl_ok = ttl_ms >= 0 && ttl_ms < ((int64_t)1 << 43);
+    B.fast = (B.ok && ttl_ok && dC >= 0 && (uint64_t)dC + fld_max <= kRelWindow) ? 1u : 0u;
+    if (B.fast) {
+        B.u0 = B.usec0 + (uint32_t)dC;
+        B.rr0 = B.r0 + (uint32_t)dC;
+        const int64_t ttlr = (int64_t)B.r0 + ttl_ms * 1000;
+        B.ttl32 = ttlr > (int64_t)0xFFFFFFFFll ? 0xFFFFFFFFu : (uint32_t)ttlr;
+    }
+    return B;
+}
+
+TBE_REL_FN uint64_t rel_row_off(int64_t t_us, const FoldRel &B) {
+    return (uint64_t)(t_us == kRelAbsent ? B.tbase : t_us) - (uint64_t)B.tbase;
+}
+TBE_REL_FN bool rel_row_slow(uint64_t off) { return off > kRelWindow; }
+
+TBE_REL_FN double rel_new_t(uint32_t u, uint32_t sec0) {
+    const uint32_t s1 = u / 1000000u;
+    const uint32_t usec = u - s1 * 1000000u;
+    const uint32_t sec = sec0 + s1;
+    const double x = (double)usec;
+    const double rcp = 1.0 / 1000000.0;
+    const double q0 = x * rcp;
+    const double r = __builtin_fma(-q0, 1000000.0, x);
+    const double q = __builtin_fma(r, rcp, q0);
+    return (double)sec + q;
+}
+
+TBE_REL_FN uint32_t rel_ms1000(uint32_t rr) { return (rr / 1000u) * 1000u; }
+TBE_REL_FN bool rel_expired(uint32_t dr, uint32_t K, uint32_t ttl32) {
+    const uint32_t bound = K > ttl32 ? K - ttl32 : 0u;
+    return dr < bound;
+}
+
+TBE_REL_FN uint32_t rel_fld(uint32_t f_lo, const FoldRel &B) { return f_lo - B.fsub; }
+TBE_REL_FN int64_t rel_grant_ts(uint32_t fld, const FoldRel &B) { return (int64_t)((uint64_t)B.tbase0 + fld); }
+
+TBE_REL_FN uint32_t fold_div_magic(uint32_t n_hi) { return (uint32_t)(((1ull << 31) + n_hi - 1) / n_hi); }
+TBE_REL_FN bool fold_div_ok(uint32_t n_hi, uint32_t grid) {
+    return n_hi >= 1 && (uint64_t)(grid >> 3) * n_hi <= (1ull << 31);
+}
+TBE_REL_FN uint32_t fold_div(uint32_t s, uint32_t m) { return (uint32_t)(((uint64_t)s * m) >> 31); }
```

After: 43.49 billion decisions/s (median of 6 runs). Within noise of the previous version (+1.0%).
